# aikiriao/LINNE

Measured on AMD Instinct MI355X. Metric: frames/sec encode (-m 7) + decode, 44.1 kHz stereo, bit-exact; 1/2/4/8 GPU, higher is better.
Workload: dtype f64; 1 GPU; encode -m 7: 1 x 60 min 44.1 kHz int16 2-channel per GPU = 15504 frames of 10240 samples (tail 9280), MS on, PCM resident in HBM; decode = inverse hot path on the encode output; frames_per_gpu=15504, channels=2, preset=7, tracks_per_gpu=1

## Files before the change

linne_amd/csrc/lnn_dev_common.h:

```cpp
#ifndef LNN_DEV_COMMON_H_INCLUDED
#define LNN_DEV_COMMON_H_INCLUDED


#include "lnn_forms.h"
typedef double lnn_d2 __attribute__((ext_vector_type(2)));
typedef int lnn_v4i __attribute__((ext_vector_type(4)));

#ifdef LNN_TIMING_EXPERIMENTS
#define LNN_DBG_IS(p, v) ((p).dbg_maxtr == (v))
#define LNN_DBG_MAXTR(p) ((p).dbg_maxtr)
#else
#define LNN_DBG_IS(p, v) false
#define LNN_DBG_MAXTR(p) 0u
#endif
struct Plan {
    uint32_t C, S, bits, L, R, ms, F, J;
    uint32_t hist;
    uint32_t rows16;
    uint32_t search_long;
    uint32_t job_off;
    uint32_t prep_general;
    uint32_t prep_defer;
    uint32_t *prep_slow_n, *prep_slow_rows;
    uint32_t fused_last;
    RowRuns runs[2];
    uint32_t P[LNN_MAXL], coef_off[LNN_MAXL];
    double regs[LNN_MAXR];
    double scale;
    const int32_t *pcm; int32_t *resid; int32_t *prm; double *stats;
    uint32_t pcm16;
    const uint32_t *cls_of_frame; const uint32_t *frame_map; const DevClass *cls; const double *sintab; const double *wtab;
    int32_t *xint, *xtmp;
    double *sig;
    double *acorr;
    double *tcoef;
    double *ptail; uint8_t *ptail_set;
    double *tloss;
    double *tsum;
    uint32_t npart;
    double *txmax;
    double *thsum;
    uint8_t *uncertain;
    uint32_t *ucount;
    unsigned long long *min_margin;
    uint32_t dbg_maxtr;
    uint32_t force_exact;
    double *lparams;
    uint32_t *lunits;
    double *jloss, *jtail;
    const double *job_reg;
    const uint32_t *af_best; const double *af_loss;
    double *af_a;
    double *af_inv;
    double *af_R;
    uint32_t af_Rstride;
    double *af_rv, *af_invd;
    double *af_obj, *af_prev;
    uint32_t *af_state;
    uint32_t *af_prob, *af_nprob;
    double *af_pivot;
    double *capture;
};
#define LNN_CAP_WORDS   8

typedef const double __attribute__((address_space(4))) *lnn_cdp;

__device__ __forceinline__ int32_t pcm24_at(const void *base, size_t i)
{
    const uint8_t *b = (const uint8_t *)base + 3u * i;
    return (int32_t)((uint32_t)b[0] | ((uint32_t)b[1] << 8)) | ((int32_t)(int8_t)b[2] << 16);
}
__device__ __forceinline__ int32_t pcm_at(const Plan &p, size_t i) { return p.pcm16 == 1u ? (int32_t)((const int16_t *)p.pcm)[i] : (p.pcm16 == 2u ? pcm24_at(p.pcm, i) : p.pcm[i]); }

__device__ __forceinline__ double round_away(double d) { return (d >= 0.0) ? floor(d + 0.5) : -floor(-d + 0.5); }
__device__ __forceinline__ int32_t mulshr5(int32_t x, int32_t c) { return (int32_t)((uint32_t)x * (uint32_t)c) >> 5; }

__device__ void levinson(const double *r, double r0, uint32_t order, double *a, double *parcor_out)
{
    for (uint32_t i = 0; i < order + 2; i++) a[i] = 0.0;
    a[0] = 1.0;
    double ek = r0;
    a[1] = -r[1] / r0;
    if (parcor_out) parcor_out[0] = r[1] / ek;
    ek += r[1] * a[1];
    for (uint32_t k = 1; k < order; k++) {
        double gamma = 0.0;
        for (uint32_t i = 0; i < k + 1; i++) gamma += a[i] * r[k + 1 - i];
        gamma /= -ek;
        ek *= (1.0 - gamma * gamma);
        const double a0 = 1.0 + gamma * 0.0;
        const double ak1 = 0.0 + gamma * 1.0;
        uint32_t i = 1, j = k;
        while (i < j) {
            const double ai = a[i], aj = a[j];
            a[i] = ai + gamma * aj;
            a[j] = aj + gamma * ai;
            i++; j--;
        }
        if (i == j) { const double ai = a[i]; a[i] = ai + gamma * ai; }
        a[0] = a0; a[k + 1] = ak1;
        if (parcor_out) parcor_out[k] = -gamma;
    }
}


#endif
```

linne_amd/csrc/lnn_device.hip:

```cpp
#include <hip/hip_runtime.h>
#include <float.h>
#include <math.h>
#include <stdint.h>
#include <stdio.h>
#include <stdlib.h>
#include <string.h>
#include <atomic>
#include <new>
#include <vector>

#include "linne_amd.h"
#include "lnn_common.h"
#include "lnn_host.h"
#include "linne_decoder.h"
#include "linne_encoder.h"

#include "lnn_dev_common.h"
#include "lnn_k_prep.h"
#include "lnn_k_autocorr.h"
#include "lnn_k_levinson.h"
#include "lnn_k_fir.h"
#include "lnn_k_search.h"
#include "lnn_k_fwdloss.h"
#include "lnn_k_lastlayer.h"
#include "lnn_k_af.h"
#include "lnn_k_train.h"
#include "lnn_k_decode.h"
#include "lnn_k_decode_rows.h"
#include "lnn_k_decode_fused.h"
#include "lnn_k_finalize.h"
#include "lnn_k_rice.h"
#include "lnn_k_stream.h"
#include "lnn_k_index_batch.h"
#include "lnn_k_windows.h"
#include "lnn_k_stream_enc.h"
#include "lnn_stream_batch.h"
#include "lnn_k_splice.h"
static_assert(LINNE_AMD_T_IB_HEADERS == 69 && LINNE_AMD_T_IB_BEHIND == 70, "the index batch's timing kinds are 69 and 70");
static_assert(LINNE_AMD_SPLICE_T_COPY == 71 && LINNE_AMD_SPLICE_T_HEADER == 72, "the splice call's timing kinds are 71 and 72");
static_assert(LNN_FIR_TILE == FIR_TILE && LNN_FIR_WAVES == FIR_THREADS / 64 && LNN_SELW_MAXPART == SELW_MAXPART && LNN_SEARCH_JOB_MIN == SEARCH_JOB_MIN && LNN_LEV_MAXRIDE == LEV_MAXRIDE, "lnn_forms.h and the kernels disagree");

#define LNN_RICE_STREAMS 4
struct LINNEAmdContext {
    int device;
    hipStream_t stream; int own_stream;
    void *arena; uint64_t arena_bytes;
    char err[256];
    int timing;
    uint32_t na_max;
    hipEvent_t ev[2]; int ev_valid;
    hipEvent_t *span_ev; int *span_kind; int nspans, span_cap;
    uint32_t *d_ucount;
    hipStream_t sub[LNN_MAXSUB]; hipEvent_t sub_done[LNN_MAXSUB]; hipEvent_t ev_start; int nsub, nsub_forced ;
    int enc_streams_done;
    hipStream_t side; hipEvent_t side_done; int has_side;
    hipStream_t sib[2]; int sib1_tried;
    hipEvent_t fork_ev[LNN_MAXSUB], join_ev[LNN_MAXSUB], lev_fork_ev[LNN_MAXSUB], lev_join_ev[LNN_MAXSUB];
    DevClass *d_cls; double *d_sin; uint64_t sin_cap; double *d_wt; uint64_t wt_cap; uint32_t *d_clsidx; uint64_t clsidx_cap; uint32_t *d_map;    uint32_t *d_nsmp; uint64_t nsmp_cap;
    LnnClassTable tab;
    int last_search_form;
    const uint32_t *cur_idx;
    uint32_t *meta_h[LNN_META]; uint64_t meta_cap[LNN_META]; hipEvent_t meta_ev[LNN_META]; int meta_used[LNN_META]; int meta_next;
    hipStream_t copy_in, copy_out; int has_copy;
    hipStream_t rice_pool[LNN_RICE_STREAMS]; int n_rice_pool, rice_next;
    uint32_t *d_plan_nsmp; uint64_t plan_nsmp_cap; double rice_steps[32]; uint32_t rice_nsteps;
    int prod_ok;
    uint32_t learning;
    uint32_t af_iters;
    double *af_h; uint32_t af_h_cap;
    int pcm16_next;
    int capture_on;
    double *d_capture; uint64_t capture_cap, capture_n;
    void *sdec; uint64_t sdec_cap;
    void *senc; uint64_t senc_cap;
    void *wdec; uint64_t wdec_cap;
    void *wstage; uint64_t wstage_cap;
    int64_t senc_count[4];
    int64_t sbatch_count[3];
    void *xcand; uint64_t xcand_cap;
    int64_t ibatch_count[5];
    int span_keep;
    double rice_guard;
    void *hstage; uint64_t hstage_cap;
    void *spl; uint64_t spl_cap;
    void *spl_stage; uint64_t spl_stage_cap;
    int64_t splice_count[6];
    int outer_keep;
    LnnKnobs knob;
};

#define HIPCHK(ctx, call) do { hipError_t e_ = (call); if (e_ != hipSuccess) { snprintf((ctx)->err, sizeof((ctx)->err), "%s:%d %s -> %s", __FILE__, __LINE__, #call, hipGetErrorString(e_)); return LNN_NG; } } while (0)

static const uint32_t k_layers_a[] = { 2, 32 }, k_layers_b[] = { 4, 64, 8 }, k_layers_c[] = { 4, 128, 16 };
static const double k_regs_1[] = { 0.0 }, k_regs_2[] = { 0.0, 1.0 / 512.0 }, k_regs_4[] = { 0.0, 1.0 / 2048.0, 1.0 / 512.0, 1.0 / 128.0 };

extern "C" int lnn_preset_info(uint32_t preset, uint32_t *num_layers, uint32_t *layers, uint32_t *num_regs, double *regs)
{
    const uint32_t *L; const double *R; uint32_t nl, nr;
    if (preset >= 8) return -1;
    if (preset < 2) { L = k_layers_a; nl = 2; } else if (preset < 5) { L = k_layers_b; nl = 3; } else { L = k_layers_c; nl = 3; }
    switch (preset) { case 0: case 2: case 5: R = k_regs_1; nr = 1; break; case 1: case 3: case 6: R = k_regs_2; nr = 2; break; default: R = k_regs_4; nr = 4; }
    if (num_layers) *num_layers = nl;
    if (layers) for (uint32_t i = 0; i < nl; i++) layers[i] = L[i];
    if (num_regs) *num_regs = nr;
    if (regs) for (uint32_t i = 0; i < nr; i++) regs[i] = R[i];
    return 0;
}

__attribute__((constructor)) static void lnn_more_hw_queues(void) { setenv("GPU_MAX_HW_QUEUES", "8", 0); }

extern "C" int LINNEAmd_GetDeviceCount(void)
{
    int n = 0;
    if (hipGetDeviceCount(&n) != hipSuccess) return 0;
    return n;
}

static int ctx_encode_streams(LINNEAmdContext *ctx)
{
    if (ctx->enc_streams_done) return LNN_OK;
    ctx->enc_streams_done = 1;
    {
        int forced = 0;
        const int ns = lnn_context_streams(&forced);
        ctx->nsub_forced = forced;
        ctx->nsub = 0;
        for (int i = 0; i < ns; i++) {
            if (hipStreamCreateWithFlags(&ctx->sub[i], hipStreamNonBlocking) != hipSuccess || hipEventCreateWithFlags(&ctx->sub_done[i], hipEventDisableTiming) != hipSuccess) break;
            ctx->nsub++;
        }
        const bool have_start = hipEventCreateWithFlags(&ctx->ev_start, hipEventDisableTiming) == hipSuccess;
        if (!have_start) ctx->nsub = 0;
        ctx->has_side = have_start && hipStreamCreateWithFlags(&ctx->side, hipStreamNonBlocking) == hipSuccess
                && hipEventCreateWithFlags(&ctx->side_done, hipEventDisableTiming) == hipSuccess;
        for (int i = 0; i < LNN_MAXSUB && ctx->has_side; i++)
            ctx->has_side = hipEventCreateWithFlags(&ctx->fork_ev[i], hipEventDisableTiming) == hipSuccess
                    && hipEventCreateWithFlags(&ctx->join_ev[i], hipEventDisableTiming) == hipSuccess
                    && hipEventCreateWithFlags(&ctx->lev_fork_ev[i], hipEventDisableTiming) == hipSuccess
                    && hipEventCreateWithFlags(&ctx->lev_join_ev[i], hipEventDisableTiming) == hipSuccess;
        if (ctx->has_side) { ctx->sib[0] = ctx->side; ctx->sib[1] = ctx->side; }
    }
    return LNN_OK;
}

extern "C" struct LINNEAmdContext *LINNEAmd_ContextCreate(int device, uint64_t scratch_bytes)
{
    int n = 0;
    hipError_t e;
#define CC_FAIL(what) do { fprintf(stderr, "liblinne_amd: ContextCreate(device=%d): %s: %s\n", device, what, hipGetErrorString(e)); } while (0)
    if ((e = hipGetDeviceCount(&n)) != hipSuccess) { CC_FAIL("hipGetDeviceCount"); return NULL; }
    if (n <= 0 || device < 0 || device >= n) { fprintf(stderr, "liblinne_amd: ContextCreate(device=%d): %d HIP device(s) visible\n", device, n); return NULL; }
    if ((e = hipSetDevice(device)) != hipSuccess) { CC_FAIL("hipSetDevice"); return NULL; }
    LINNEAmdContext *ctx = (LINNEAmdContext *)calloc(1, sizeof(*ctx));
    if (!ctx) return NULL;
    ctx->device = device;
    if ((e = hipStreamCreateWithFlags(&ctx->stream, hipStreamNonBlocking)) != hipSuccess) { CC_FAIL("hipStreamCreate"); free(ctx); return NULL; }
    ctx->own_stream = 1;
    if (scratch_bytes == 0) scratch_bytes = 6ull << 30;
    if ((e = hipMalloc(&ctx->arena, scratch_bytes)) != hipSuccess) { CC_FAIL("hipMalloc(arena)"); hipStreamDestroy(ctx->stream); free(ctx); return NULL; }
    ctx->arena_bytes = scratch_bytes;
    if ((e = hipMalloc((void **)&ctx->d_cls, sizeof(DevClass) * LNN_MAXCLS)) != hipSuccess) { CC_FAIL("hipMalloc(classes)"); hipFree(ctx->arena); hipStreamDestroy(ctx->stream); free(ctx); return NULL; }
    if ((e = hipMalloc((void **)&ctx->d_ucount, 4 * sizeof(uint32_t))) != hipSuccess) { CC_FAIL("hipMalloc(counter)"); }
    lnn_knobs_read_context(&ctx->knob); ctx->last_search_form = -1;
    (void)hipFuncSetAttribute((const void *)k_levinson_lds, hipFuncAttributeMaxDynamicSharedMemorySize, (int)LEV_LDS_BUDGET);
    (void)hipFuncSetAttribute((const void *)k_synth_pipe, hipFuncAttributeMaxDynamicSharedMemorySize, (int)LEV_LDS_BUDGET);
    if ((e = hipEventCreate(&ctx->ev[0])) != hipSuccess || (e = hipEventCreate(&ctx->ev[1])) != hipSuccess) { CC_FAIL("hipEventCreate"); }
#undef CC_FAIL
    return ctx;
}

extern "C" void LINNEAmd_ContextDestroy(struct LINNEAmdContext *ctx)
{
    if (!ctx) return;
    hipSetDevice(ctx->device);
    hipStreamSynchronize(ctx->stream);
    if (ctx->arena) hipFree(ctx->arena);
    if (ctx->d_cls) hipFree(ctx->d_cls);
    if (ctx->d_ucount) hipFree(ctx->d_ucount);
    if (ctx->d_capture) hipFree(ctx->d_capture);
    for (int i = 0; i < ctx->nsub; i++) { hipStreamSynchronize(ctx->sub[i]); hipStreamDestroy(ctx->sub[i]); hipEventDestroy(ctx->sub_done[i]); }
    if (ctx->ev_start) hipEventDestroy(ctx->ev_start);
    if (ctx->has_side && ctx->sib[1] != ctx->side) { hipStreamSynchronize(ctx->sib[1]); hipStreamDestroy(ctx->sib[1]); }
    if (ctx->has_side) { hipStreamSynchronize(ctx->side); hipStreamDestroy(ctx->side); hipEventDestroy(ctx->side_done); }
    for (int i = 0; i < LNN_MAXSUB; i++) {
        if (ctx->fork_ev[i]) hipEventDestroy(ctx->fork_ev[i]);
        if (ctx->join_ev[i]) hipEventDestroy(ctx->join_ev[i]);
        if (ctx->lev_fork_ev[i]) hipEventDestroy(ctx->lev_fork_ev[i]);
        if (ctx->lev_join_ev[i]) hipEventDestroy(ctx->lev_join_ev[i]);
    }
    if (ctx->d_sin) hipFree(ctx->d_sin);
    if (ctx->d_wt) hipFree(ctx->d_wt);
    if (ctx->d_clsidx) hipFree(ctx->d_clsidx);
    if (ctx->d_nsmp) hipFree(ctx->d_nsmp);
    if (ctx->d_plan_nsmp) hipFree(ctx->d_plan_nsmp);
    if (ctx->hstage) hipFree(ctx->hstage);
    if (ctx->sdec) hipFree(ctx->sdec);
    if (ctx->senc) hipFree(ctx->senc);
    if (ctx->wdec) hipFree(ctx->wdec);
    if (ctx->xcand) hipFree(ctx->xcand);
    if (ctx->spl) hipFree(ctx->spl);
    if (ctx->spl_stage) hipHostFree(ctx->spl_stage);
    if (ctx->wstage) hipHostFree(ctx->wstage);
    if (ctx->af_h) hipHostFree(ctx->af_h);
    for (int i = 0; i < LNN_META; i++) { if (ctx->meta_h[i]) hipHostFree(ctx->meta_h[i]); if (ctx->meta_ev[i]) hipEventDestroy(ctx->meta_ev[i]); }
    for (int i = 0; i < ctx->n_rice_pool; i++) { hipStreamSynchronize(ctx->rice_pool[i]); hipStreamDestroy(ctx->rice_pool[i]); }
    if (ctx->has_copy) { hipStreamSynchronize(ctx->copy_in); hipStreamSynchronize(ctx->copy_out); hipStreamDestroy(ctx->copy_in); hipStreamDestroy(ctx->copy_out); }
    hipEventDestroy(ctx->ev[0]); hipEventDestroy(ctx->ev[1]);
    for (int i = 0; i < 2 * ctx->span_cap; i++) hipEventDestroy(ctx->span_ev[i]);
    free(ctx->span_ev); free(ctx->span_kind);
    if (ctx->own_stream) hipStreamDestroy(ctx->stream);
    free(ctx);
}

extern "C" const char *LINNEAmd_GetLastError(const struct LINNEAmdContext *ctx) { return ctx ? ctx->err : "no context"; }

extern "C" int LINNEAmd_SetStream(struct LINNEAmdContext *ctx, void *hip_stream)
{
    if (!ctx) return LNN_INVALID_ARGUMENT;
    HIPCHK(ctx, hipSetDevice(ctx->device));
    HIPCHK(ctx, hipStreamSynchronize(ctx->stream));
    if (ctx->own_stream) { HIPCHK(ctx, hipStreamDestroy(ctx->stream)); ctx->own_stream = 0; }
    ctx->stream = (hipStream_t)hip_stream;
    return LNN_OK;
}

extern "C" int LINNEAmd_ReserveScratch(struct LINNEAmdContext *ctx, uint64_t bytes)
{
    if (!ctx) return LNN_INVALID_ARGUMENT;
    if (ctx->arena_bytes >= bytes) return LNN_OK;
    HIPCHK(ctx, hipSetDevice(ctx->device));
    HIPCHK(ctx, hipStreamSynchronize(ctx->stream));
    void *fresh = NULL;
    if (hipMalloc(&fresh, bytes) != hipSuccess) { (void)hipGetLastError(); snprintf(ctx->err, sizeof(ctx->err), "cannot reserve %llu bytes of scratch", (unsigned long long)bytes); return LNN_NG; }
    if (ctx->arena) HIPCHK(ctx, hipFree(ctx->arena));
    ctx->arena = fresh; ctx->arena_bytes = bytes;
    return LNN_OK;
}

extern "C" int64_t LINNEAmd_GetLastFallbackCount(struct LINNEAmdContext *ctx)
{
    if (!ctx) return -1;
    uint32_t v = 0;
    if (hipSetDevice(ctx->device) != hipSuccess || hipStreamSynchronize(ctx->stream) != hipSuccess
            || hipMemcpy(&v, ctx->d_ucount, sizeof(v), hipMemcpyDeviceToHost) != hipSuccess) return -1;
    return (int64_t)v;
}

extern "C" double LINNEAmd_GetLastMinMargin(struct LINNEAmdContext *ctx)
{
    if (!ctx) return -1.0;
    double v = -1.0;
    if (hipSetDevice(ctx->device) != hipSuccess || hipStreamSynchronize(ctx->stream) != hipSuccess
            || hipMemcpy(&v, ctx->d_ucount + 2, sizeof(v), hipMemcpyDeviceToHost) != hipSuccess) return -1.0;
    return v;
}

extern "C" int LINNEAmd_SetSearchCapture(struct LINNEAmdContext *ctx, int enable)
{
    if (!ctx) return LNN_INVALID_ARGUMENT;
    ctx->capture_on = enable ? 1 : 0;
    return LNN_OK;
}

extern "C" int64_t LINNEAmd_GetLastSearchCapture(struct LINNEAmdContext *ctx, double *host, uint64_t capacity_records)
{
    if (!ctx) return -1;
    const uint64_t n = ctx->capture_n < capacity_records ? ctx->capture_n : capacity_records;
    if (hipSetDevice(ctx->device) != hipSuccess || hipStreamSynchronize(ctx->stream) != hipSuccess) return -1;
    if (n && (!host || hipMemcpy(host, ctx->d_capture, n * LNN_CAP_WORDS * sizeof(double), hipMemcpyDeviceToHost) != hipSuccess)) return -1;
    return (int64_t)ctx->capture_n;
}

extern "C" int LINNEAmd_Synchronize(struct LINNEAmdContext *ctx)
{
    if (!ctx) return LNN_INVALID_ARGUMENT;
    HIPCHK(ctx, hipSetDevice(ctx->device));
    HIPCHK(ctx, hipStreamSynchronize(ctx->stream));
    return LNN_OK;
}

extern "C" int LINNEAmd_SetLearning(struct LINNEAmdContext *ctx, uint32_t enable)
{
    if (!ctx) return LNN_INVALID_ARGUMENT;
    ctx->learning = enable ? 1u : 0u;
    return LNN_OK;
}
extern "C" int LINNEAmd_SetAfIterations(struct LINNEAmdContext *ctx, uint32_t iterations)
{
    if (!ctx) return LNN_INVALID_ARGUMENT;
    ctx->af_iters = iterations;
    return LNN_OK;
}
extern "C" int LINNEAmd_EnableTiming(struct LINNEAmdContext *ctx, int enable) { if (!ctx) return LNN_INVALID_ARGUMENT; ctx->timing = enable; return LNN_OK; }
static int span_begin(LINNEAmdContext *ctx, int kind, hipStream_t st)
{
    if (!ctx->timing) return -1;
    if (ctx->nspans == ctx->span_cap) {
        const int ncap = ctx->span_cap ? ctx->span_cap * 2 : 256;
        hipEvent_t *ne = (hipEvent_t *)realloc(ctx->span_ev, sizeof(hipEvent_t) * 2 * ncap);
        if (!ne) return -1;
        ctx->span_ev = ne;
        int *nk = (int *)realloc(ctx->span_kind, sizeof(int) * ncap);
        if (!nk) return -1;
        ctx->span_kind = nk;
        for (int i = 2 * ctx->span_cap; i < 2 * ncap; i++) if (hipEventCreate(&ctx->span_ev[i]) != hipSuccess) return -1;
        ctx->span_cap = ncap;
    }
    const int id = ctx->nspans++;
    ctx->span_kind[id] = kind;
    (void)hipEventRecord(ctx->span_ev[2 * id], st);
    return id;
}
static void span_end(LINNEAmdContext *ctx, int id, hipStream_t st) { if (id >= 0) (void)hipEventRecord(ctx->span_ev[2 * id + 1], st); }

extern "C" double LINNEAmd_GetLastTimingMs(struct LINNEAmdContext *ctx, int which)
{
    if (!ctx || which < 0) return -1.0;
    if (which == 0) {
        float ms = -1.0f;
        if (!ctx->ev_valid) return -1.0;
        if (hipEventSynchronize(ctx->ev[1]) != hipSuccess || hipEventElapsedTime(&ms, ctx->ev[0], ctx->ev[1]) != hipSuccess) return -1.0;
        return ms;
    }
    double sum = 0.0; int cnt = 0;
    for (int i = 0; i < ctx->nspans; i++) if (ctx->span_kind[i] == which) {
        float ms = 0.0f;
        if (hipEventSynchronize(ctx->span_ev[2 * i + 1]) != hipSuccess || hipEventElapsedTime(&ms, ctx->span_ev[2 * i], ctx->span_ev[2 * i + 1]) != hipSuccess) return -1.0;
        sum += ms; cnt++;
    }
    return cnt ? sum : -1.0;
}
extern "C" int LINNEAmd_GetLastSearchLongForm(struct LINNEAmdContext *ctx) { return ctx ? ctx->last_search_form : -1; }
extern "C" int LINNEAmd_GetLastTimingLaunches(struct LINNEAmdContext *ctx, int which)
{
    if (!ctx) return 0;
    int cnt = 0;
    for (int i = 0; i < ctx->nspans; i++) if (ctx->span_kind[i] == which) cnt++;
    return cnt;
}

static int ensure_buf(LINNEAmdContext *ctx, void **ptr, uint64_t *cap, uint64_t need)
{
    if (*cap >= need) return LNN_OK;
    HIPCHK(ctx, hipStreamSynchronize(ctx->stream));
    if (*ptr) HIPCHK(ctx, hipFree(*ptr));
    *ptr = NULL; *cap = 0;
    HIPCHK(ctx, hipMalloc(ptr, need));
    *cap = need;
    return LNN_OK;
}

static int shape_info(const struct LINNEAmdShape *s, HostShape *h)
{
    if (!s || s->preset >= 8 || s->num_channels == 0 || s->num_channels > LNN_MAXCH || s->bits_per_sample == 0 || s->bits_per_sample > 32
            || s->num_samples_per_block == 0 || s->ch_process_method > 1 || (s->ch_process_method == 1 && s->num_channels < 2)) return LNN_INVALID_FORMAT;
    lnn_preset_info(s->preset, &h->L, h->P, &h->R, h->regs);
    uint32_t off = 0; h->maxP = 0;
    for (uint32_t l = 0; l < h->L; l++) { h->coef_off[l] = off; off += h->P[l]; if (h->P[l] > h->maxP) h->maxP = h->P[l]; }
    for (uint32_t l = 0; l < h->L; l++) if (s->num_samples_per_block <= h->P[l]) return LNN_INVALID_FORMAT;
    return LNN_OK;
}

static int meta_acquire(LINNEAmdContext *ctx, uint32_t F, int *m_out)
{
    const int m = ctx->meta_next;
    ctx->meta_next = (m + 1) % LNN_META;
    if (ctx->meta_used[m]) { HIPCHK(ctx, hipEventSynchronize(ctx->meta_ev[m])); ctx->meta_used[m] = 0; }
    if (!ctx->meta_ev[m]) HIPCHK(ctx, hipEventCreateWithFlags(&ctx->meta_ev[m], hipEventDisableTiming));
    if (ctx->meta_cap[m] < 4ull * F) {
        const uint64_t cap = 4ull * (F < 4096u ? 4096u : F);
        if (ctx->meta_h[m]) { HIPCHK(ctx, hipHostFree(ctx->meta_h[m])); ctx->meta_h[m] = NULL; ctx->meta_cap[m] = 0; }
        HIPCHK(ctx, hipHostMalloc((void **)&ctx->meta_h[m], sizeof(uint32_t) * cap, hipHostMallocDefault));
        ctx->meta_cap[m] = cap;
    }
    *m_out = m;
    return LNN_OK;
}

static int copy_lengths(LINNEAmdContext *ctx, const struct LINNEAmdShape *shape, const uint32_t *h_num_samples, uint32_t F, uint32_t *dst)
{
    const uint32_t S = shape->num_samples_per_block;
    for (uint32_t f = 0; f < F; f++) {
        const uint32_t n = h_num_samples ? h_num_samples[f] : S;
        if (n == 0 || n > S) { snprintf(ctx->err, sizeof(ctx->err), "frame %u: num_samples %u out of range", f, n); return LNN_INVALID_ARGUMENT; }
        dst[f] = n;
    }
    return LNN_OK;
}

static int upload_lengths(LINNEAmdContext *ctx, const struct LINNEAmdShape *shape, const uint32_t *h_num_samples, uint32_t F)
{
    int m, ret;
    if ((ret = meta_acquire(ctx, F, &m)) != LNN_OK) return ret;
    uint32_t *nsm = ctx->meta_h[m];
    if ((ret = copy_lengths(ctx, shape, h_num_samples, F, nsm)) != LNN_OK) return ret;
    if ((ret = ensure_buf(ctx, (void **)&ctx->d_nsmp, &ctx->nsmp_cap, sizeof(uint32_t) * (uint64_t)(F ? F : 1))) != LNN_OK) return ret;
    HIPCHK(ctx, hipMemcpyAsync(ctx->d_nsmp, nsm, sizeof(uint32_t) * F, hipMemcpyHostToDevice, ctx->stream));
    HIPCHK(ctx, hipEventRecord(ctx->meta_ev[m], ctx->stream));
    ctx->meta_used[m] = 1;
    return LNN_OK;
}

extern "C" double lnn_welch_divisor(uint32_t unit_samples) { return lnn_welch_div(unit_samples); }
extern "C" double lnn_sin_window(uint32_t s, uint32_t n) { return sin((3.1415926535897932384626433832795029 * s) / (n - 1)); }
extern "C" double lnn_cholesky_pivot(double sum) { return pow(sum, -0.5); }

static int build_classes(LINNEAmdContext *ctx, const struct LINNEAmdShape *shape, const HostShape *hs,
        const uint32_t *h_num_samples, uint32_t F)
{
    int m, ret;
    { const int r_ = meta_acquire(ctx, F, &m); if (r_ != LNN_OK) return r_; }
    uint32_t *idx = ctx->meta_h[m], *map = ctx->meta_h[m] + F, *raw = ctx->meta_h[m] + 2 * (size_t)F;
    ctx->cur_idx = idx;
    LnnClassTable &tab = ctx->tab;
    LnnCallClasses cc;
    switch (lnn_call_classes(&tab, shape, hs, &ctx->knob, h_num_samples, F, idx, map, raw, &cc)) {
    case LNN_CLS_BAD_LENGTH: snprintf(ctx->err, sizeof(ctx->err), "frame %u: num_samples %u out of range", cc.error_frame, h_num_samples[cc.error_frame]); return LNN_INVALID_ARGUMENT;
    case LNN_CLS_TOO_MANY: snprintf(ctx->err, sizeof(ctx->err), "more than %d distinct frame lengths in one batch", LNN_MAXCLS); return LNN_INVALID_ARGUMENT;
    default: break;
    }
    ctx->na_max = cc.na_max; ctx->prod_ok = cc.prod_ok;
    if (cc.branch != LNN_CLS_REUSE) {
        const uint64_t sin_total = tab.sin_total, wt_total = tab.wt_total;
        double *sintab = (double *)malloc(sizeof(double) * (sin_total ? sin_total : 1));
        double *wt = (double *)calloc(wt_total ? wt_total : 1, sizeof(double));
        if (!sintab || !wt) { free(sintab); free(wt); tab.valid = 0; tab.ncls = 0; snprintf(ctx->err, sizeof(ctx->err), "out of host memory"); return LNN_NG; }
        for (uint32_t k = 0; k < tab.ncls; k++) {
            const DevClass &c = tab.cls[k];
            const uint32_t n = c.n;
            for (uint32_t s = 0; s < n; s++) sintab[c.sin_off + s] = lnn_sin_window(s, n);
            for (uint32_t l = 0; l < hs->L; l++)
                for (uint32_t t = 0; t < c.ntrials[l]; t++) {
                    const uint32_t u = c.trial_u[l][t], nu = c.na / u;
                    const double div = c.trial_div[l][t];
                    double *w = wt + c.wt_off[l][t];
                    for (uint32_t loc = 0; loc < nu; loc++) {
                        const uint32_t h = (loc < (nu >> 1)) ? loc : (nu - 1 - loc);
                        w[loc] = div * (double)h * (double)(nu - 1 - h);
                    }
                }
        }
        hipError_t e = hipDeviceSynchronize();
        ret = (e == hipSuccess) ? ensure_buf(ctx, (void **)&ctx->d_sin, &ctx->sin_cap, sizeof(double) * (sin_total ? sin_total : 1)) : LNN_NG;
        if (ret == LNN_OK) ret = ensure_buf(ctx, (void **)&ctx->d_wt, &ctx->wt_cap, sizeof(double) * (wt_total ? wt_total : 1));
        if (ret != LNN_OK) { free(sintab); free(wt); tab.valid = 0; tab.ncls = 0; return ret; }
        e = hipMemcpyAsync(ctx->d_sin, sintab, sizeof(double) * sin_total, hipMemcpyHostToDevice, ctx->stream);
        if (e == hipSuccess) e = hipMemcpyAsync(ctx->d_wt, wt, sizeof(double) * wt_total, hipMemcpyHostToDevice, ctx->stream);
        if (e == hipSuccess) e = hipMemcpyAsync(ctx->d_cls, tab.cls, sizeof(DevClass) * LNN_MAXCLS, hipMemcpyHostToDevice, ctx->stream);
        if (e == hipSuccess) e = hipStreamSynchronize(ctx->stream);
        free(sintab); free(wt);
        if (e != hipSuccess) { tab.valid = 0; tab.ncls = 0; snprintf(ctx->err, sizeof(ctx->err), "class table upload: %s", hipGetErrorString(e)); return LNN_NG; }
    }
    if ((ret = ensure_buf(ctx, (void **)&ctx->d_clsidx, &ctx->clsidx_cap, sizeof(uint32_t) * 2 * (uint64_t)(F ? F : 1))) != LNN_OK) return ret;
    ctx->d_map = ctx->d_clsidx + F;
    HIPCHK(ctx, hipMemcpyAsync(ctx->d_clsidx, idx, sizeof(uint32_t) * 2 * (size_t)F, hipMemcpyHostToDevice, ctx->stream));
    HIPCHK(ctx, hipEventRecord(ctx->meta_ev[m], ctx->stream));
    ctx->meta_used[m] = 1;
    return LNN_OK;
}

static uint64_t align_up(uint64_t v) { return (v + 255u) & ~(uint64_t)255u; }

static uint64_t frame_scratch_bytes(const struct LINNEAmdShape *shape, const HostShape *hs, uint32_t af_iters = 0, uint32_t learning = 0)
{
    const uint64_t C = shape->num_channels, S = shape->num_samples_per_block, J = C * hs->R;
    uint64_t b = 0;
    b += 2 * C * S * sizeof(int32_t);
    b += J * 2 * S * sizeof(double);
    b += J * LNN_MAXT * LNN_ACW * sizeof(double);
    b += J * LNN_MAXT * LNN_MAXP * sizeof(double);
    b += J * LNN_MAXT * LNN_MAXU * (sizeof(double) + 1);
    b += J * LNN_MAXT * sizeof(double) * (1 + (uint64_t)((S + FIR_TILE - 1) / FIR_TILE) * (FIR_THREADS / 64)) + J;
    b += J * sizeof(double) * (uint64_t)((S + FIR_TILE - 1) / FIR_TILE) * (FIR_THREADS / 64) + 256;
    b += J * LNN_MAXT * sizeof(double) + 256;
    b += J * LNN_MAXL * LNN_MAXP * sizeof(double);
    b += J * LNN_MAXL * sizeof(uint32_t);
    b += J * 2 * sizeof(double);
    b += C * sizeof(uint32_t) + 512;
    if (af_iters)
        b += C * (sizeof(double) * ((uint64_t)hs->maxP * hs->maxP + S + 3 * LNN_MAXP + 3 * LNN_MAXU + 2) + sizeof(uint32_t) * (2 * LNN_MAXU + 1)) + 8192;
    if (af_iters || learning) b += C * (sizeof(uint32_t) + 2 * sizeof(double)) + 1024;
    if (learning)
        b += C * (sizeof(double) * ((2 + LNN_MAXL) * S + 2 * LNN_MAXL * LNN_MAXP + 2) + sizeof(uint32_t)) + 4096;
    return b + 4096;
}

extern "C" uint64_t LINNEAmd_ScratchBytesPerFrame(const struct LINNEAmdShape *shape)
{
    HostShape hs;
    if (shape_info(shape, &hs) != LNN_OK) return 0;
    return frame_scratch_bytes(shape, &hs);
}

#define LNN_BY_ORDER(P_, LAUNCH_) do { switch (P_) { case 2: LAUNCH_(2); break; case 4: LAUNCH_(4); break; case 8: LAUNCH_(8); break; default: LAUNCH_(16); break; } } while (0)
#define LNN_BY_L0_SPEC(l0_, spec_, LAUNCH_) do { if (l0_) { if (spec_) LAUNCH_(true, true); else LAUNCH_(true, false); } else { if (spec_) LAUNCH_(false, true); else LAUNCH_(false, false); } } while (0)

template <int MODE> static void launch_fir(hipStream_t st, const Plan &p, uint32_t l, uint32_t cur, uint32_t J, uint32_t grid_y, bool spec)
{
    const dim3 grid(J, grid_y), blk(FIR_THREADS);
#define LNN_F2(L0_, SPEC_) hipLaunchKernelGGL((k_fir2<MODE, L0_, SPEC_>), grid, blk, 0, st, p, l, cur)
    LNN_BY_L0_SPEC(l == 0, spec, LNN_F2);
#undef LNN_F2
}

template <int PP> static void launch_fir_small_p(hipStream_t st, const Plan &p, uint32_t l, uint32_t cur, const dim3 grid, bool spec)
{
#define LNN_FS(L0_, SPEC_) hipLaunchKernelGGL((k_fir_small<PP, L0_, SPEC_>), grid, dim3(FIR_THREADS), 0, st, p, l, cur)
    LNN_BY_L0_SPEC(l == 0, spec, LNN_FS);
#undef LNN_FS
}
static void launch_fir_small_search(hipStream_t st, const Plan &p, uint32_t l, uint32_t cur, uint32_t J, uint32_t tiles, bool spec, uint32_t P)
{
    const dim3 grid(l == 0 ? J / p.R : J, tiles);
#define LNN_FSP(PP_) launch_fir_small_p<PP_>(st, p, l, cur, grid, spec)
    LNN_BY_ORDER(P, LNN_FSP);
#undef LNN_FSP
}

static void launch_last_layer(hipStream_t st, const Plan &q, uint32_t l, uint32_t cur, uint32_t J)
{
#define LNN_LL(PP_) hipLaunchKernelGGL(k_last_layer<PP_>, dim3((J + 63) / 64), dim3(64), 0, st, q, l, cur)
    LNN_BY_ORDER(q.P[l], LNN_LL);
#undef LNN_LL
}

static void launch_fwd_loss(hipStream_t st, const Plan &q, uint32_t l, uint32_t cur, uint32_t J, bool mw)
{
    const dim3 g((J + 63) / 64);
#define LNN_FLM(PP_) hipLaunchKernelGGL(k_fwd_loss_mw<PP_>, g, dim3(320), 0, st, q, l, cur)
#define LNN_FL(PP_) hipLaunchKernelGGL(k_fwd_loss<PP_>, g, dim3(64), 0, st, q, l, cur)
    if (mw) LNN_BY_ORDER(q.P[l], LNN_FLM); else LNN_BY_ORDER(q.P[l], LNN_FL);
#undef LNN_FLM
#undef LNN_FL
}

static void launch_search_long(hipStream_t st, const Plan &q, uint32_t l, uint32_t cur, uint32_t J, uint32_t tiles, int form)
{
    const dim3 grid(J, form == 2 ? 1u : tiles), blk(FIR_THREADS);
#define LNN_SL(TWO_, JOB_) do { if (q.P[l] == 128u) hipLaunchKernelGGL((k_search_long<128, TWO_, JOB_>), grid, blk, 0, st, q, l, cur); else hipLaunchKernelGGL((k_search_long<64, TWO_, JOB_>), grid, blk, 0, st, q, l, cur); } while (0)
    if (form == 2) LNN_SL(true, true); else if (form == 1) LNN_SL(true, false); else LNN_SL(false, false);
#undef LNN_SL
}

struct EncodeCall {
    const struct LINNEAmdShape *shape; HostShape hs; uint32_t C, S, num_frames, pcm16;
    const int32_t *d_pcm; int32_t *d_residual, *d_params; double *d_stats;
    LnnSplit split;
};
struct Chunk {
    LINNEAmdContext *ctx; hipStream_t st; const HostShape *hs;
    hipStream_t sib; uint32_t slot;
    uint32_t C, S, f0, Fc; uint64_t CF, J;
    const uint32_t *idx;
    Plan p; LnnChunkForms forms;
    uint8_t *abase; uint64_t part_bytes;
    uint32_t *af_best; double *af_loss, *af_reg; TrainArgs tr;
};
struct Pass {
    const Plan *q; const LnnChunkForms *forms; uint32_t J, af_iters;
    uint32_t cur;
};

static void fill_plan(Plan &p, const EncodeCall &e, uint32_t F)
{
    memset(&p, 0, sizeof(p));
    p.C = e.C; p.S = e.S; p.bits = e.shape->bits_per_sample; p.L = e.hs.L; p.R = e.hs.R; p.F = F;
    for (uint32_t l = 0; l < e.hs.L; l++) p.P[l] = e.hs.P[l];
    p.scale = ldexp(1.0, -(int)(e.shape->bits_per_sample - 1));
    p.pcm = e.d_pcm; p.pcm16 = e.pcm16; p.stats = e.d_stats;
}

static int launch_stats(LINNEAmdContext *ctx, const EncodeCall &e)
{
    Plan ps; fill_plan(ps, e, e.num_frames);
    ps.cls_of_frame = ctx->d_clsidx; ps.frame_map = ctx->d_map; ps.cls = ctx->d_cls; ps.sintab = ctx->d_sin;
    hipStream_t ss = ctx->stream;
    if (ctx->has_side) { ss = ctx->side; HIPCHK(ctx, hipStreamWaitEvent(ss, ctx->ev_start, 0)); }
    if (!ctx->knob.nostats) {
        const int sp_ = span_begin(ctx, LINNE_AMD_T_STATS, ss);
        if (lnn_stats_rows_form(&ctx->knob, e.num_frames, e.C, e.S, e.hs.P[0])) {
            const dim3 g((e.num_frames * e.C + 63u) / 64u);
#define LNN_SR(W_, T_) do { if (e.pcm16 == 1u) hipLaunchKernelGGL((k_stats_rows<W_, 1>), g, dim3(T_), 0, ss, ps); else if (e.pcm16 == 2u) hipLaunchKernelGGL((k_stats_rows<W_, 2>), g, dim3(T_), 0, ss, ps); else hipLaunchKernelGGL((k_stats_rows<W_, 0>), g, dim3(T_), 0, ss, ps); } while (0)
            if (e.hs.P[0] == 4u) LNN_SR(5, 320); else LNN_SR(3, 192);
#undef LNN_SR
        }
        else hipLaunchKernelGGL(k_stats, dim3(e.num_frames, e.C), dim3(STAT_THREADS), 0, ss, ps);
        span_end(ctx, sp_, ss);
    }
    if (ss != ctx->stream) HIPCHK(ctx, hipEventRecord(ctx->side_done, ss));
    return LNN_OK;
}

static int chunk_setup(Chunk &k, LINNEAmdContext *ctx, const EncodeCall &e, uint32_t f0, uint32_t slot)
{
    const uint32_t S = e.S;
    k.ctx = ctx; k.hs = &e.hs; k.C = e.C; k.S = S; k.f0 = f0;
    k.st = e.split.use_sub ? ctx->sub[slot] : ctx->stream;
    k.slot = slot; k.sib = ctx->sib[slot & 1u];
    k.Fc = (e.num_frames - f0 < e.split.chunk) ? (e.num_frames - f0) : (uint32_t)e.split.chunk;
    k.CF = (uint64_t)k.Fc * e.C; k.J = k.CF * e.hs.R;
    k.idx = ctx->cur_idx + f0;
    const uint64_t CF = k.CF, J = k.J;
    const LnnChunkIn in = { &e.hs, e.C, S, k.Fc, ctx->tab.cls, k.idx, &ctx->knob, e.split.use_sub, ctx->has_side != 0, ctx->af_iters, ctx->learning, false };
    lnn_chunk_forms(&in, &k.forms);
    Plan &p = k.p;
    fill_plan(p, e, k.Fc);
    p.ms = e.shape->ch_process_method; p.J = (uint32_t)J;
    for (uint32_t l = 0; l < e.hs.L; l++) p.coef_off[l] = e.hs.coef_off[l];
    for (uint32_t r = 0; r < e.hs.R; r++) p.regs[r] = e.hs.regs[r];
    p.resid = e.d_residual; p.prm = e.d_params;
    p.fused_last = k.forms.fuse_cfg ? 1u : 0u;
    p.search_long = ctx->knob.search_long ? 1u : 0u;
    p.rows16 = ctx->knob.rows16 ? 1u : 0u;
    p.prep_general = ctx->knob.prep_general ? 1u : 0u;
    p.prep_defer = k.forms.prep_defer ? 1u : 0u;
    lnn_build_runs(&p.runs[0], k.idx, k.Fc, e.C); lnn_build_runs(&p.runs[1], k.idx, k.Fc, e.C * e.hs.R);
    p.hist = k.forms.hist ? 1u : 0u;
    p.cls_of_frame = ctx->d_clsidx + f0; p.frame_map = ctx->d_map + f0; p.cls = ctx->d_cls; p.sintab = ctx->d_sin; p.wtab = ctx->d_wt; p.ucount = ctx->d_ucount; p.min_margin = (unsigned long long *)(ctx->d_ucount + 2); p.force_exact = ctx->knob.force_exact ? 1u : 0u; p.dbg_maxtr = ctx->knob.dbg_maxtr;
    p.capture = ctx->capture_n ? ctx->d_capture : NULL;
    k.part_bytes = e.split.part_bytes;
    k.abase = (uint8_t *)ctx->arena + (size_t)slot * k.part_bytes;
    uint8_t *a = k.abase;
#define TAKE(ptr, type, count) do { ptr = (type *)a; a += align_up(sizeof(type) * (uint64_t)(count)); } while (0)
    TAKE(p.xint, int32_t, CF * S); TAKE(p.xtmp, int32_t, CF * S);
    TAKE(p.sig, double, J * 2 * S);
    TAKE(p.acorr, double, J * LNN_MAXT * LNN_ACW); TAKE(p.tcoef, double, J * LNN_MAXT * LNN_MAXP);
    TAKE(p.ptail, double, J * LNN_MAXT * LNN_MAXU); TAKE(p.ptail_set, uint8_t, J * LNN_MAXT * LNN_MAXU);
    TAKE(p.tloss, double, J * LNN_MAXT); p.npart = ((S + FIR_TILE - 1) / FIR_TILE) * (FIR_THREADS / 64); TAKE(p.tsum, double, J * LNN_MAXT * p.npart); TAKE(p.txmax, double, J * p.npart); TAKE(p.thsum, double, J * LNN_MAXT); TAKE(p.uncertain, uint8_t, J); TAKE(p.lparams, double, J * LNN_MAXL * LNN_MAXP);
    TAKE(p.lunits, uint32_t, J * LNN_MAXL); TAKE(p.jloss, double, J); TAKE(p.jtail, double, J);
    TAKE(p.prep_slow_n, uint32_t, 64); TAKE(p.prep_slow_rows, uint32_t, CF);
    k.af_best = NULL; k.af_loss = NULL; k.af_reg = NULL;
    memset(&k.tr, 0, sizeof(k.tr));
    TrainArgs &tr = k.tr;
    if (ctx->af_iters || ctx->learning) { TAKE(k.af_best, uint32_t, CF); TAKE(k.af_loss, double, CF); TAKE(k.af_reg, double, CF); }
    if (ctx->learning) {
        TAKE(tr.buf, double, CF * TR_NBUF * S); TAKE(tr.dparams, double, CF * LNN_MAXL * LNN_MAXP); TAKE(tr.momentum, double, CF * LNN_MAXL * LNN_MAXP);
        TAKE(tr.loss, double, CF); TAKE(tr.prev, double, CF); TAKE(tr.active, uint32_t, CF); TAKE(tr.nactive, uint32_t, 64);
    }
    if (ctx->af_iters) {
        TAKE(p.af_a, double, CF * LNN_MAXP); TAKE(p.af_inv, double, CF * S); p.af_Rstride = e.hs.maxP * e.hs.maxP; TAKE(p.af_R, double, CF * p.af_Rstride);
        TAKE(p.af_rv, double, CF * LNN_MAXP); TAKE(p.af_invd, double, CF * LNN_MAXP);
        TAKE(p.af_obj, double, CF * LNN_MAXU); TAKE(p.af_prev, double, CF * LNN_MAXU); TAKE(p.af_state, uint32_t, CF * LNN_MAXU);
        TAKE(p.af_prob, uint32_t, CF * LNN_MAXU); TAKE(p.af_nprob, uint32_t, 64); TAKE(p.af_pivot, double, CF * LNN_MAXU);
    }
#undef TAKE
    if ((uint64_t)(a - k.abase) > k.part_bytes) { snprintf(ctx->err, sizeof(ctx->err), "internal: arena overflow"); return LNN_NG; }
    return LNN_OK;
}

static int launch_prep(Chunk &k)
{
    LINNEAmdContext *ctx = k.ctx; hipStream_t st = k.st; const Plan &p = k.p;
    if (p.prep_defer) HIPCHK(ctx, hipMemsetAsync(p.prep_slow_n, 0, sizeof(uint32_t), st));
    const int sp_ = span_begin(ctx, LINNE_AMD_T_PREP, st);
    hipLaunchKernelGGL(k_prep, dim3(k.Fc, k.C), dim3(PREP_THREADS), 0, st, p);
    if (p.prep_defer) hipLaunchKernelGGL(k_prep_slow, dim3((uint32_t)((k.CF + 63) / 64)), dim3(256), 0, st, p);
    span_end(ctx, sp_, st);
    return LNN_OK;
}

static void sibling_for_levinson(Chunk &k)
{
    LINNEAmdContext *ctx = k.ctx;
    if ((k.slot & 1u) && ctx->sib[1] == ctx->side && !ctx->sib1_tried) {
        ctx->sib1_tried = 1;
        if (hipStreamCreateWithFlags(&ctx->sib[1], hipStreamNonBlocking) != hipSuccess) { (void)hipGetLastError(); ctx->sib[1] = ctx->side; }
    }
    k.sib = ctx->sib[k.slot & 1u];
}

static int launch_lags(Chunk &k, const Pass &ps, uint32_t l)
{
    LINNEAmdContext *ctx = k.ctx; hipStream_t st = k.st; const Plan &q = *ps.q; const LnnLayerForms &lf = ps.forms->layer[l];
    const uint32_t P = k.hs->P[l];
    if (lf.lev_beside && !lf.lev_inline) sibling_for_levinson(k);
    if (lf.beside) {
        HIPCHK(ctx, hipEventRecord(ctx->fork_ev[k.slot], st)); HIPCHK(ctx, hipStreamWaitEvent(k.sib, ctx->fork_ev[k.slot], 0));
        const int sp_ = span_begin(ctx, LINNE_AMD_T_AUTOCORR, k.sib); dispatch_autocorr2(k.sib, q, l, ps.cur, ctx->na_max, (ctx->prod_ok >> l) & 1); span_end(ctx, sp_, k.sib);
        HIPCHK(ctx, hipEventRecord(ctx->join_ev[k.slot], k.sib));
    }
    if (lf.hist_layer) {
        for (int w = 0; w < 3; w++) {
            if (P == 64u && w == 1) continue;
            const int sp_ = span_begin(ctx, LINNE_AMD_T_HIST_P + w, st); (void)launch_autocorr_hist(st, q, l, ps.cur, w, w == 2 && lf.lev_beside); span_end(ctx, sp_, st);
            if (w == 0 && lf.lev_beside) {
                const LnnLevLaunch &v = lf.lev[0];
                const hipStream_t ls = lf.lev_inline ? st : k.sib;
                if (lf.lev_inline && lf.beside) HIPCHK(ctx, hipStreamWaitEvent(st, ctx->join_ev[k.slot], 0));
                if (!lf.lev_inline) { HIPCHK(ctx, hipEventRecord(ctx->lev_fork_ev[k.slot], st)); HIPCHK(ctx, hipStreamWaitEvent(k.sib, ctx->lev_fork_ev[k.slot], 0)); }
                hipLaunchKernelGGL(k_levinson_lds, dim3((ps.J + 63) / 64, v.u), dim3(v.threads), v.lds, ls, q, l, v.t, v.ride);
                if (!lf.lev_inline) HIPCHK(ctx, hipEventRecord(ctx->lev_join_ev[k.slot], k.sib));
            }
        }
    }
    if (lf.beside) HIPCHK(ctx, hipStreamWaitEvent(st, ctx->join_ev[k.slot], 0));
    else if (!lf.hist_all) {
        const int sp_ = span_begin(ctx, (P >= 32u) ? LINNE_AMD_T_AUTOCORR : LINNE_AMD_T_AUTOCORR_SHORT, st); dispatch_autocorr2(st, q, l, ps.cur, ctx->na_max, (ctx->prod_ok >> l) & 1); span_end(ctx, sp_, st);
    }
    return LNN_OK;
}

static void launch_levinson(Chunk &k, const Pass &ps, uint32_t l)
{
    LINNEAmdContext *ctx = k.ctx; hipStream_t st = k.st; const Plan &q = *ps.q; const LnnLayerForms &lf = ps.forms->layer[l];
    const uint32_t P = k.hs->P[l], maxu = P < 128u ? P : 128u;
    if (lf.lev_beside && !lf.lev_inline) (void)hipStreamWaitEvent(st, ctx->lev_join_ev[k.slot], 0);
    const int sp_ = span_begin(ctx, LINNE_AMD_T_LEVINSON, st);
    if (lf.lev_wave) hipLaunchKernelGGL(k_levinson_wave, dim3(ps.J, 2u * maxu - 1u), dim3(64), 0, st, q, l);
    else for (uint32_t i = lf.lev_beside ? 1u : 0u; i < lf.nlev; i++) {
        const LnnLevLaunch &v = lf.lev[i];
        hipLaunchKernelGGL(k_levinson_lds, dim3((ps.J + 63) / 64, v.u), dim3(v.threads), v.lds, st, q, l, v.t, v.ride);
    }
    span_end(ctx, sp_, st);
}

static void launch_search(Chunk &k, const Pass &ps, uint32_t l)
{
    LINNEAmdContext *ctx = k.ctx; hipStream_t st = k.st; const Plan &q = *ps.q; const LnnLayerForms &lf = ps.forms->layer[l];
    const uint32_t tiles = (k.S + FIR_TILE - 1) / FIR_TILE;
    if (lf.long_any) {
        const int sp_ = span_begin(ctx, LINNE_AMD_T_SEARCH_LONG, st);
        ctx->last_search_form = lf.search_form == 2 ? 1 : 0;
        launch_search_long(st, q, l, ps.cur, ps.J, tiles, lf.search_form);
        span_end(ctx, sp_, st);
    }
    if (lf.long_any && lf.long_all) return;
    const int sp_ = span_begin(ctx, (l == 0) ? LINNE_AMD_T_SEARCH_L0 : (lf.fir_spec ? LINNE_AMD_T_SEARCH : LINNE_AMD_T_SEARCH_PLAIN), st);
    if (lf.fir_small) launch_fir_small_search(st, q, l, ps.cur, ps.J, tiles, lf.fir_spec, k.hs->P[l]);
    else if (lf.long_any) {
        const uint32_t rpf = ps.J / k.Fc;
        for (uint32_t f = 0, g = 0; lnn_next_left_run(&lf, k.idx, k.Fc, g, &f, &g); ) {
            Plan qq = q; qq.job_off = f * rpf;
            launch_fir<2>(st, qq, l, ps.cur, (g - f) * rpf, tiles, lf.fir_spec);
        }
    }
    else launch_fir<2>(st, q, l, ps.cur, ps.J, tiles, lf.fir_spec);
    span_end(ctx, sp_, st);
}

static void launch_select(Chunk &k, const Pass &ps, uint32_t l)
{
    LINNEAmdContext *ctx = k.ctx; hipStream_t st = k.st; const Plan &q = *ps.q; const LnnLayerForms &lf = ps.forms->layer[l];
    for (uint32_t exact = 0; exact < 2; exact++) {
        const int sp_ = span_begin(ctx, exact ? LINNE_AMD_T_EXACT : LINNE_AMD_T_SELECT, st);
        if (exact) { if (l == 0) hipLaunchKernelGGL((k_fir2<0, true, false>), dim3(ps.J, 1), dim3(FIR_THREADS), 0, st, q, l, ps.cur); else hipLaunchKernelGGL((k_fir2<0, false, false>), dim3(ps.J, 1), dim3(FIR_THREADS), 0, st, q, l, ps.cur); }
        if (lf.sel_wave) hipLaunchKernelGGL(k_select_wave, dim3(ps.J), dim3(64), 0, st, q, l, exact);
        else hipLaunchKernelGGL(k_select, dim3((ps.J + 63) / 64), dim3(64), 0, st, q, l, exact);
        span_end(ctx, sp_, st);
    }
}

static int run_af(Chunk &k, const Pass &ps, uint32_t l)
{
    LINNEAmdContext *ctx = k.ctx; hipStream_t st = k.st; const Plan &q = *ps.q;
    const uint32_t P = k.hs->P[l], S = k.S, Jq = ps.J, cur = ps.cur;
    HIPCHK(ctx, hipMemsetAsync(q.af_nprob, 0, sizeof(uint32_t), st));
    hipLaunchKernelGGL(k_af_init, dim3((Jq + 255) / 256), dim3(256), 0, st, q, l);
    uint32_t nprob = 0;
    HIPCHK(ctx, hipMemcpyAsync(&nprob, q.af_nprob, sizeof(uint32_t), hipMemcpyDeviceToHost, st));
    HIPCHK(ctx, hipStreamSynchronize(st));
    if (nprob == 0) return LNN_OK;
    if (ctx->af_h_cap < nprob) {
        if (ctx->af_h) HIPCHK(ctx, hipHostFree(ctx->af_h));
        ctx->af_h = NULL; ctx->af_h_cap = 0;
        HIPCHK(ctx, hipHostMalloc((void **)&ctx->af_h, sizeof(double) * (size_t)nprob, hipHostMallocDefault));
        ctx->af_h_cap = nprob;
    }
    uint32_t mblocks = 0;
    for (uint32_t uu = 1; uu <= P; uu <<= 1) { const uint32_t b_ = uu * afm_blocks_per_unit(P / uu); if (b_ > mblocks) mblocks = b_; }
    for (uint32_t it = 0; it < ps.af_iters; it++) {
        hipLaunchKernelGGL(k_af_resid, dim3(Jq, (S + AFR_THREADS * 4 - 1) / (AFR_THREADS * 4)), dim3(AFR_THREADS), 0, st, q, l, cur);
        hipLaunchKernelGGL(k_af_obj, dim3(nprob), dim3(64), 0, st, q, l, cur);
        hipLaunchKernelGGL(k_af_matrix, dim3(Jq, mblocks), dim3(AFM_THREADS), 0, st, q, l, cur);
        for (uint32_t i = 0; i < P; i++) {
            hipLaunchKernelGGL(k_af_pivot, dim3((nprob + 63) / 64), dim3(64), 0, st, q, l, i);
            HIPCHK(ctx, hipMemcpyAsync(ctx->af_h, q.af_pivot, sizeof(double) * (size_t)nprob, hipMemcpyDeviceToHost, st));
            HIPCHK(ctx, hipStreamSynchronize(st));
            for (uint32_t j = 0; j < nprob; j++) { const double v = ctx->af_h[j]; ctx->af_h[j] = (v <= 0.0) ? -1.0 : lnn_cholesky_pivot(v); }
            HIPCHK(ctx, hipMemcpyAsync(q.af_pivot, ctx->af_h, sizeof(double) * (size_t)nprob, hipMemcpyHostToDevice, st));
            hipLaunchKernelGGL(k_af_column, dim3(nprob), dim3(128), 0, st, q, l, i);
        }
        hipLaunchKernelGGL(k_af_solve, dim3((nprob + 63) / 64), dim3(64), 0, st, q, l);
    }
    hipLaunchKernelGGL(k_af_finish, dim3((Jq + 255) / 256), dim3(256), 0, st, q, l);
    HIPCHK(ctx, hipGetLastError());
    return LNN_OK;
}

static int run_layers(Chunk &k, Pass &ps)
{
    LINNEAmdContext *ctx = k.ctx; hipStream_t st = k.st; const Plan &q = *ps.q;
    const uint32_t L = k.hs->L, tiles = (k.S + FIR_TILE - 1) / FIR_TILE;
    int ret;
    ps.cur = 0;
    for (uint32_t l = 0; l < L; l++) {
        const LnnLayerForms &lf = ps.forms->layer[l];
        if ((ret = launch_lags(k, ps, l)) != LNN_OK) return ret;
        launch_levinson(k, ps, l);
        if (lf.last_layer) {
            { const int sp_ = span_begin(ctx, LINNE_AMD_T_FWD_LOSS, st); launch_last_layer(st, q, l, ps.cur, ps.J); span_end(ctx, sp_, st); }
            { const int sp_ = span_begin(ctx, LINNE_AMD_T_SELECT, st); hipLaunchKernelGGL(k_select, dim3((ps.J + 63) / 64), dim3(64), 0, st, q, l, 2u); span_end(ctx, sp_, st); }
        } else {
            launch_search(k, ps, l);
            launch_select(k, ps, l);
            if (lf.fwd_loss) { const int sp_ = span_begin(ctx, LINNE_AMD_T_FWD_LOSS, st); launch_fwd_loss(st, q, l, ps.cur, ps.J, lf.fwd_loss_mw); span_end(ctx, sp_, st); }
        }
        if (ps.af_iters && (ret = run_af(k, ps, l)) != LNN_OK) return ret;
        if (lf.forward) {
            const int sp_ = span_begin(ctx, (l == 0) ? LINNE_AMD_T_FORWARD_L0 : (lf.fir_spec ? LINNE_AMD_T_FORWARD : LINNE_AMD_T_FORWARD_PLAIN), st);
            launch_fir<1>(st, q, l, ps.cur, ps.J, lf.forward_walk ? 1u : tiles, lf.fir_spec);
            span_end(ctx, sp_, st);
        }
        ps.cur ^= 1u;
    }
    return LNN_OK;
}

static int run_train(Chunk &k, const Plan &q, const uint32_t *best)
{
    LINNEAmdContext *ctx = k.ctx; hipStream_t st = k.st; TrainArgs &tr = k.tr;
    const uint32_t CF = (uint32_t)k.CF, L = k.hs->L;
    tr.p = q; tr.best = best; tr.CF = CF;
    const uint32_t tiles = (k.S + TR_TILE - 1) / TR_TILE;
    const int sp_ = span_begin(ctx, LINNE_AMD_T_TRAIN, st);
    hipLaunchKernelGGL(k_tr_init, dim3((CF + 255) / 256), dim3(256), 0, st, tr);
    for (uint32_t it = 0; it < 2000u; it++) {
        HIPCHK(ctx, hipMemsetAsync(tr.nactive, 0, sizeof(uint32_t), st));
        for (uint32_t l = 0; l < L; l++) hipLaunchKernelGGL(k_tr_forward, dim3(CF, tiles), dim3(TR_THREADS), 0, st, tr, l);
        hipLaunchKernelGGL(k_tr_loss, dim3(CF), dim3(64), 0, st, tr);
        for (uint32_t l = L - 1; l >= 1; l--) hipLaunchKernelGGL(k_tr_back, dim3(CF, tiles), dim3(TR_THREADS), 0, st, tr, l);
        hipLaunchKernelGGL(k_tr_gradp, dim3(CF, L), dim3(128), 0, st, tr);
        hipLaunchKernelGGL(k_tr_update, dim3(CF), dim3(128), 0, st, tr, (double)0.8f, (double)0.1f, 1.0e-7);
        uint32_t left = 0;
        HIPCHK(ctx, hipMemcpyAsync(&left, tr.nactive, sizeof(uint32_t), hipMemcpyDeviceToHost, st));
        HIPCHK(ctx, hipStreamSynchronize(st));
        if (left == 0) break;
    }
    span_end(ctx, sp_, st);
    HIPCHK(ctx, hipGetLastError());
    return LNN_OK;
}

static void launch_finish(Chunk &k, const Plan &q)
{
    const uint32_t CF = (uint32_t)k.CF;
    const int sp_ = span_begin(k.ctx, LINNE_AMD_T_FINALIZE, k.st);
    hipLaunchKernelGGL(k_quantize, dim3(CF), dim3(64), 0, k.st, q);
    hipLaunchKernelGGL(k_fir_cascade, dim3(CF, k.forms.cascade_walk ? 1u : (k.S + FIN_TILE - 1) / FIN_TILE), dim3(FIN_THREADS), 0, k.st, q);
    span_end(k.ctx, sp_, k.st);
}

static int run_final_pass(Chunk &k)
{
    LINNEAmdContext *ctx = k.ctx; hipStream_t st = k.st; const Plan &p = k.p;
    const uint32_t CF = (uint32_t)k.CF;
    int ret;
    Plan q = p;
    q.R = 1; q.J = CF; q.regs[0] = 0.0;
    q.hist = 0; q.fused_last = 0; q.search_long = 0;
    q.capture = NULL;
    lnn_build_runs(&q.runs[1], k.idx, k.Fc, k.C);
    q.job_reg = k.af_reg; q.af_best = k.af_best; q.af_loss = k.af_loss;
    hipLaunchKernelGGL(k_af_best, dim3((CF + 255) / 256), dim3(256), 0, st, p, k.af_best, k.af_loss, k.af_reg);
    const LnnChunkIn in = { k.hs, k.C, k.S, k.Fc, ctx->tab.cls, k.idx, &ctx->knob, false, ctx->has_side != 0, ctx->af_iters, ctx->learning, true };
    LnnChunkForms ff;
    lnn_chunk_forms(&in, &ff);
    Pass fp = { &q, &ff, CF, ctx->af_iters, 0 };
    const int sp_ = span_begin(ctx, LINNE_AMD_T_AF_PASS, st);
    if ((ret = run_layers(k, fp)) != LNN_OK) return ret;
    span_end(ctx, sp_, st);
    if (ctx->learning && (ret = run_train(k, q, NULL)) != LNN_OK) return ret;
    launch_finish(k, q);
    return LNN_OK;
}

static int enqueue_chunk(Chunk &k)
{
    LINNEAmdContext *ctx = k.ctx; hipStream_t st = k.st; const Plan &p = k.p;
    int ret;
    if ((ret = launch_prep(k)) != LNN_OK) return ret;
    Pass sp = { &p, &k.forms, (uint32_t)k.J, 0u, 0 };
    if ((ret = run_layers(k, sp)) != LNN_OK) return ret;
    if (k.forms.chain_sum) {
        const int sp_ = span_begin(ctx, LINNE_AMD_T_FINAL_LOSS, st);
        if (k.forms.chain_sum_wave) hipLaunchKernelGGL(k_chain_sum_wave<1>, dim3((uint32_t)k.J), dim3(64), 0, st, p, 0u, sp.cur);
        else hipLaunchKernelGGL(k_chain_sum<1>, dim3(((uint32_t)k.J + 63) / 64), dim3(SUM_THREADS), 0, st, p, 0u, sp.cur);
        span_end(ctx, sp_, st);
    }
    if (ctx->af_iters) { if ((ret = run_final_pass(k)) != LNN_OK) return ret; }
    else {
        if (ctx->learning) {
            hipLaunchKernelGGL(k_af_best, dim3(((uint32_t)k.CF + 255) / 256), dim3(256), 0, st, p, k.af_best, k.af_loss, k.af_reg);
            if ((ret = run_train(k, p, k.af_best)) != LNN_OK) return ret;
        }
        launch_finish(k, p);
    }
    HIPCHK(ctx, hipGetLastError());
    return LNN_OK;
}

static int enqueue_chunks(LINNEAmdContext *ctx, const EncodeCall &e)
{
    uint32_t chunk_index = 0;
    for (uint32_t f0 = 0; f0 < e.num_frames; f0 += (uint32_t)e.split.chunk, chunk_index++) {
        Chunk k;
        int ret = chunk_setup(k, ctx, e, f0, chunk_index % e.split.nsub);
        if (ret == LNN_OK) ret = enqueue_chunk(k);
        if (ret != LNN_OK) return ret;
    }
    return LNN_OK;
}

extern "C" int LINNEAmd_EncodeFramesDevice(struct LINNEAmdContext *ctx, const struct LINNEAmdShape *shape,
        const int32_t *d_pcm, const uint32_t *h_num_samples, uint32_t num_frames,
        int32_t *d_residual, int32_t *d_params, double *d_stats)
{
    if (!ctx) return LNN_INVALID_ARGUMENT;
    ctx->err[0] = 0;
    EncodeCall e;
    e.pcm16 = (uint32_t)ctx->pcm16_next;
    ctx->pcm16_next = 0;
    if (!shape || !d_pcm || !d_residual || !d_params || !d_stats) { snprintf(ctx->err, sizeof(ctx->err), "null argument"); return LNN_INVALID_ARGUMENT; }
    if (num_frames == 0) return LNN_OK;
    int ret = shape_info(shape, &e.hs);
    if (ret != LNN_OK) { snprintf(ctx->err, sizeof(ctx->err), "invalid shape"); return ret; }
    e.shape = shape; e.C = shape->num_channels; e.S = shape->num_samples_per_block; e.num_frames = num_frames;
    e.d_pcm = d_pcm; e.d_residual = d_residual; e.d_params = d_params; e.d_stats = d_stats;
    HIPCHK(ctx, hipSetDevice(ctx->device));
    if ((ret = ctx_encode_streams(ctx)) != LNN_OK) return ret;
    lnn_knobs_read_call(&ctx->knob);
    if ((ret = build_classes(ctx, shape, &e.hs, h_num_samples, num_frames)) != LNN_OK) return ret;
    const uint64_t per_frame = frame_scratch_bytes(shape, &e.hs, ctx->af_iters, ctx->learning);
    if (ctx->arena_bytes < per_frame * 4 + 65536) {
        HIPCHK(ctx, hipStreamSynchronize(ctx->stream));
        HIPCHK(ctx, hipFree(ctx->arena)); ctx->arena = NULL; ctx->arena_bytes = 0;
        HIPCHK(ctx, hipMalloc(&ctx->arena, per_frame * 4 + 65536));
        ctx->arena_bytes = per_frame * 4 + 65536;
    }
    e.split = lnn_call_split(ctx->arena_bytes, per_frame, num_frames, e.C, e.hs.R, ctx->nsub, ctx->nsub_forced != 0, &ctx->knob);
    const LnnSplit &sp = e.split;
    if (!ctx->span_keep) ctx->nspans = 0;
    ctx->last_search_form = -1;
    ctx->capture_n = 0;
    if (ctx->capture_on) {
        const uint64_t nrec = (uint64_t)num_frames * e.C * e.hs.R * e.hs.L * LNN_MAXT;
        if (ctx->capture_cap < nrec) {
            HIPCHK(ctx, hipStreamSynchronize(ctx->stream));
            if (ctx->d_capture) HIPCHK(ctx, hipFree(ctx->d_capture));
            ctx->d_capture = NULL; ctx->capture_cap = 0;
            HIPCHK(ctx, hipMalloc((void **)&ctx->d_capture, nrec * LNN_CAP_WORDS * sizeof(double)));
            ctx->capture_cap = nrec;
        }
        HIPCHK(ctx, hipMemsetAsync(ctx->d_capture, 0xFF, nrec * LNN_CAP_WORDS * sizeof(double), ctx->stream));
        ctx->capture_n = nrec;
    }
    HIPCHK(ctx, hipMemsetAsync(ctx->d_ucount, 0, sizeof(uint32_t), ctx->stream));
    HIPCHK(ctx, hipMemsetAsync(ctx->d_ucount + 2, 0x7F, 2 * sizeof(uint32_t), ctx->stream));
    if (ctx->timing && !ctx->span_keep) { HIPCHK(ctx, hipEventRecord(ctx->ev[0], ctx->stream)); }
    if (sp.use_sub || ctx->has_side) HIPCHK(ctx, hipEventRecord(ctx->ev_start, ctx->stream));
    if (sp.use_sub) for (uint32_t i = 0; i < sp.nsub; i++) HIPCHK(ctx, hipStreamWaitEvent(ctx->sub[i], ctx->ev_start, 0));
    if ((ret = launch_stats(ctx, e)) != LNN_OK) return ret;
    const int loop_ret = enqueue_chunks(ctx, e);
    if (loop_ret != LNN_OK) {
        if (sp.use_sub) for (uint32_t i = 0; i < sp.nsub; i++) (void)hipStreamSynchronize(ctx->sub[i]);
        if (ctx->has_side) { (void)hipStreamSynchronize(ctx->side); (void)hipStreamSynchronize(ctx->sib[1]); }
        return loop_ret;
    }
    if (ctx->has_side) HIPCHK(ctx, hipStreamWaitEvent(ctx->stream, ctx->side_done, 0));
    if (sp.use_sub) {
        for (uint32_t i = 0; i < sp.nsub; i++) { HIPCHK(ctx, hipEventRecord(ctx->sub_done[i], ctx->sub[i])); HIPCHK(ctx, hipStreamWaitEvent(ctx->stream, ctx->sub_done[i], 0)); }
    }
    if (ctx->timing) { HIPCHK(ctx, hipEventRecord(ctx->ev[1], ctx->stream)); ctx->ev_valid = 1; }
    return LNN_OK;
}

static int params_in_range(LINNEAmdContext *ctx, const HostShape *hs, uint32_t C, const int32_t *h_params, uint32_t num_frames)
{
    uint32_t ncoef = 0;
    for (uint32_t l = 0; l < hs->L; l++) ncoef += hs->P[l];
    const uint64_t rows = (uint64_t)num_frames * C;
    uint32_t bad = 0;
    for (uint64_t r = 0; r < rows; r++) {
        const int32_t *c = h_params + r * LINNE_AMD_PARAM_WORDS + LINNE_AMD_PRM_COEF;
        uint32_t acc = 0;
        for (uint32_t i = 0; i < ncoef; i++) acc |= (uint32_t)(c[i] + 128) & ~255u;
        bad |= acc;
    }
    if (bad) { snprintf(ctx->err, sizeof(ctx->err), "a coefficient outside [-128, 127] in the parameter records (not a LINNE stream's)"); return LNN_INVALID_FORMAT; }
    return LNN_OK;
}

static void launch_synth_rows(hipStream_t st, const DecPlan &p, uint32_t l, const LnnDecLayer &d, uint32_t CF)
{
    const dim3 grows((CF + 3) / 4), grows8((CF + 7) / 8), b(64);
    if (d.form == LNN_DL_ROWS8) switch (d.pb) {
    case 4: hipLaunchKernelGGL((k_synth_rows8<4>), grows8, b, 0, st, p, l); break;
    case 8: hipLaunchKernelGGL((k_synth_rows8<8>), grows8, b, 0, st, p, l); break;
    default: hipLaunchKernelGGL((k_synth_rows8<16>), grows8, b, 0, st, p, l); break;
    }
    else switch (d.nch) {
    case 0: if (d.pb == 4u) hipLaunchKernelGGL((k_synth_rows<0, 4>), grows, b, 0, st, p, l); else hipLaunchKernelGGL((k_synth_rows<0>), grows, b, 0, st, p, l); break;
    case 1: hipLaunchKernelGGL((k_synth_rows<1>), grows, b, 0, st, p, l); break;
    case 3: hipLaunchKernelGGL((k_synth_rows<3>), grows, b, 0, st, p, l); break;
    default: hipLaunchKernelGGL((k_synth_rows<7>), grows, b, 0, st, p, l); break;
    }
}
template <int PP> static void launch_synth_small_p(hipStream_t st, const DecPlan &p, uint32_t l, bool de, uint32_t CF)
{
    if (de) hipLaunchKernelGGL((k_synth_small<PP, true>), dim3((CF + 63) / 64), dim3(64), 0, st, p, l); else hipLaunchKernelGGL((k_synth_small<PP, false>), dim3((CF + 63) / 64), dim3(64), 0, st, p, l);
}
static void launch_synth_lanes(hipStream_t st, const DecPlan &p, uint32_t l, const LnnDecLayer &d, uint32_t CF)
{
#define LNN_SS(PP_) launch_synth_small_p<PP_>(st, p, l, d.de, CF)
    if (d.form == LNN_DL_SMALL) LNN_BY_ORDER(d.pb, LNN_SS);
#undef LNN_SS
    else if (d.form == LNN_DL_BIG) switch (d.pb) {
    case 32:  hipLaunchKernelGGL((k_synth_big<32>), dim3((CF + 15) / 16), dim3(64), 0, st, p, l); break;
    case 64:  hipLaunchKernelGGL((k_synth_big<64>), dim3((CF + 15) / 16), dim3(64), 0, st, p, l); break;
    default: hipLaunchKernelGGL((k_synth_big<128>), dim3((CF + 15) / 16), dim3(64), 0, st, p, l); break;
    }
    else hipLaunchKernelGGL(k_synthesize, dim3(CF), dim3(64), 0, st, p, l, 0u);
}

static int decode_frames_dev(LINNEAmdContext *ctx, const struct LINNEAmdShape *shape, const HostShape &hs,
        int32_t *d_data, const uint32_t *d_nsmp, uint32_t num_frames, const int32_t *d_params)
{
    DecPlan p; memset(&p, 0, sizeof(p));
    p.C = shape->num_channels; p.S = shape->num_samples_per_block; p.L = hs.L; p.ms = shape->ch_process_method; p.F = num_frames;
    for (uint32_t l = 0; l < hs.L; l++) { p.P[l] = hs.P[l]; p.coef_off[l] = hs.coef_off[l]; }
    p.data = d_data; p.prm = d_params; p.nsmp = d_nsmp;
    hipStream_t st = ctx->stream;
    const uint32_t CF = num_frames * p.C, gsmall = (CF + 63) / 64;
    if (hs.P[0] > 16) { snprintf(ctx->err, sizeof(ctx->err), "internal: layer 0 of order %u", hs.P[0]); return LNN_NG; }
    LnnDecodeForms df;
    lnn_decode_forms(&hs, p.C, p.S, p.ms, num_frames, ((uintptr_t)d_data & 15u) == 0u, SP_LDS_BYTES(p.S) <= LEV_LDS_BUDGET, &ctx->knob, &df);
    if (df.call == LNN_DEC_PIPE) { const int sp_ = span_begin(ctx, LINNE_AMD_T_SYNTH_PIPE, st); hipLaunchKernelGGL(k_synth_pipe, dim3(CF), dim3(64 * (hs.L + 1)), SP_LDS_BYTES(p.S), st, p); span_end(ctx, sp_, st); }
    else if (df.call == LNN_DEC_WAVE) { const int sp_ = span_begin(ctx, LINNE_AMD_T_SYNTH, st); hipLaunchKernelGGL(k_synthesize, dim3(CF), dim3(64), 0, st, p, 0xFFFFFFFFu, 1u); span_end(ctx, sp_, st); }
    else for (int32_t li = (int32_t)hs.L - 1; li >= 0; li--) {
        const uint32_t l = (uint32_t)li;
        const LnnDecLayer &d = df.layer[l];
        if (d.form == LNN_DL_FUSED_L0) {
            const int sp_ = span_begin(ctx, LINNE_AMD_T_SYNTH_L0_DE, st);
            if (d.ms_fold) hipLaunchKernelGGL((k_synth_l0_de<true>), dim3(gsmall), dim3(64 * SF_WAVES), 0, st, p); else hipLaunchKernelGGL((k_synth_l0_de<false>), dim3(gsmall), dim3(64 * SF_WAVES), 0, st, p);
            span_end(ctx, sp_, st);
        } else if (d.form == LNN_DL_ROWS || d.form == LNN_DL_ROWS8) {
            const int sp_ = span_begin(ctx, d.nch > 0 ? LINNE_AMD_T_SYNTH_ROWS : LINNE_AMD_T_SYNTH_ROWS_SHORT, st);
            launch_synth_rows(st, p, l, d, CF);
            span_end(ctx, sp_, st);
            if (d.de) {
                const int sd_ = span_begin(ctx, LINNE_AMD_T_DEEMPH_LR, st);
                if (d.ms_fold) hipLaunchKernelGGL((k_deemph_lr<true>), dim3(gsmall), dim3(64 * (2 + DL_STORERS)), 0, st, p); else hipLaunchKernelGGL((k_deemph_lr<false>), dim3(gsmall), dim3(64 * (2 + DL_STORERS)), 0, st, p);
                span_end(ctx, sd_, st);
            }
        } else {
            const int sp_ = span_begin(ctx, d.form == LNN_DL_SMALL ? LINNE_AMD_T_SYNTH_SMALL : (d.form == LNN_DL_BIG ? LINNE_AMD_T_SYNTH_BIG : LINNE_AMD_T_SYNTH), st);
            launch_synth_lanes(st, p, l, d, CF);
            span_end(ctx, sp_, st);
        }
    }
    if (df.ms_separate)
        { const int sp_ = span_begin(ctx, LINNE_AMD_T_MS_TO_LR, st); hipLaunchKernelGGL(k_ms_to_lr, dim3(num_frames, (p.S + 255) / 256), dim3(256), 0, st, p); span_end(ctx, sp_, st); }
    HIPCHK(ctx, hipGetLastError());
    if (ctx->timing) { HIPCHK(ctx, hipEventRecord(ctx->ev[1], ctx->stream)); ctx->ev_valid = 1; }
    return LNN_OK;
}

extern "C" int LINNEAmd_DecodeFramesDevice(struct LINNEAmdContext *ctx, const struct LINNEAmdShape *shape,
        int32_t *d_data, const uint32_t *h_num_samples, uint32_t num_frames, const int32_t *d_params)
{
    if (!ctx) return LNN_INVALID_ARGUMENT;
    ctx->err[0] = 0;
    if (!shape || !d_data || !d_params) { snprintf(ctx->err, sizeof(ctx->err), "null argument"); return LNN_INVALID_ARGUMENT; }
    if (num_frames == 0) return LNN_OK;
    HostShape hs;
    int ret = shape_info(shape, &hs);
    if (ret != LNN_OK) { snprintf(ctx->err, sizeof(ctx->err), "invalid shape"); return ret; }
    HIPCHK(ctx, hipSetDevice(ctx->device));
    lnn_knobs_read_call(&ctx->knob);
    if ((ret = upload_lengths(ctx, shape, h_num_samples, num_frames)) != LNN_OK) return ret;
    ctx->nspans = 0;
    if (ctx->timing) { HIPCHK(ctx, hipEventRecord(ctx->ev[0], ctx->stream)); }
    return decode_frames_dev(ctx, shape, hs, d_data, ctx->d_nsmp, num_frames, d_params);
}

#define HSTAGE_KEEP ((uint64_t)64 << 20)
static int hstage_get(LINNEAmdContext *ctx, uint64_t bytes, void **out, int *transient)
{
    *transient = 0;
    if (bytes > HSTAGE_KEEP) {
        if (hipMalloc(out, bytes) != hipSuccess) { (void)hipGetLastError(); snprintf(ctx->err, sizeof(ctx->err), "hipMalloc of staging buffers failed"); return LNN_NG; }
        *transient = 1;
        return LNN_OK;
    }
    if (ctx->hstage_cap < bytes) {
        HIPCHK(ctx, hipStreamSynchronize(ctx->stream));
        if (ctx->hstage) { HIPCHK(ctx, hipFree(ctx->hstage)); ctx->hstage = NULL; ctx->hstage_cap = 0; }
        uint64_t cap = bytes < ((uint64_t)1 << 20) ? ((uint64_t)1 << 20) : bytes;
        if (hipMalloc(&ctx->hstage, cap) != hipSuccess) { (void)hipGetLastError(); ctx->hstage = NULL; snprintf(ctx->err, sizeof(ctx->err), "hipMalloc of staging buffers failed"); return LNN_NG; }
        ctx->hstage_cap = cap;
    }
    *out = ctx->hstage;
    return LNN_OK;
}

extern "C" int LINNEAmd_EncodeFramesHost(struct LINNEAmdContext *ctx, const struct LINNEAmdShape *shape,
        const int32_t *pcm, const uint32_t *num_samples, uint32_t num_frames,
        int32_t *residual, int32_t *params, double *stats)
{
    if (!ctx) return LNN_INVALID_ARGUMENT;
    if (!shape || !pcm || !residual || !params || !stats) return LNN_INVALID_ARGUMENT;
    if (num_frames == 0) return LNN_OK;
    HIPCHK(ctx, hipSetDevice(ctx->device));
    const uint64_t CS = (uint64_t)shape->num_channels * shape->num_samples_per_block;
    const uint64_t nb = sizeof(int32_t) * CS * num_frames, pb = sizeof(int32_t) * LINNE_AMD_PARAM_WORDS * (uint64_t)shape->num_channels * num_frames,
                   sb = sizeof(double) * LINNE_AMD_STAT_WORDS * (uint64_t)shape->num_channels * num_frames;
    int32_t *d_pcm = NULL, *d_res = NULL, *d_prm = NULL; double *d_st = NULL;
    void *stage = NULL; int transient = 0;
    const uint64_t nb_a = align_up(nb), pb_a = align_up(pb);
    int ret = hstage_get(ctx, 2 * nb_a + pb_a + align_up(sb), &stage, &transient);
    if (ret != LNN_OK) return ret;
    d_pcm = (int32_t *)stage; d_res = (int32_t *)((uint8_t *)stage + nb_a); d_prm = (int32_t *)((uint8_t *)stage + 2 * nb_a); d_st = (double *)((uint8_t *)stage + 2 * nb_a + pb_a);
    ret = LNN_NG;
    if (hipMemcpyAsync(d_pcm, pcm, nb, hipMemcpyHostToDevice, ctx->stream) != hipSuccess) { snprintf(ctx->err, sizeof(ctx->err), "H2D failed"); goto done; }
    if (hipMemsetAsync(d_prm, 0, pb, ctx->stream) != hipSuccess || hipMemsetAsync(d_st, 0, sb, ctx->stream) != hipSuccess) { snprintf(ctx->err, sizeof(ctx->err), "memset failed"); goto done; }
    ret = LINNEAmd_EncodeFramesDevice(ctx, shape, d_pcm, num_samples, num_frames, d_res, d_prm, d_st);
    if (ret != LNN_OK) goto done;
    ret = LNN_NG;
    if (hipMemcpyAsync(residual, d_res, nb, hipMemcpyDeviceToHost, ctx->stream) != hipSuccess
            || hipMemcpyAsync(params, d_prm, pb, hipMemcpyDeviceToHost, ctx->stream) != hipSuccess
            || hipMemcpyAsync(stats, d_st, sb, hipMemcpyDeviceToHost, ctx->stream) != hipSuccess) { snprintf(ctx->err, sizeof(ctx->err), "D2H failed"); goto done; }
    {
        hipError_t e = hipStreamSynchronize(ctx->stream);
        if (e != hipSuccess) { snprintf(ctx->err, sizeof(ctx->err), "stream sync: %s", hipGetErrorString(e)); goto done; }
    }
    ret = LNN_OK;
done:
    if (ret != LNN_OK || transient) hipStreamSynchronize(ctx->stream);
    if (transient) hipFree(stage);
    return ret;
}

extern "C" int LINNEAmd_DecodeFramesHost(struct LINNEAmdContext *ctx, const struct LINNEAmdShape *shape,
        int32_t *data, const uint32_t *num_samples, uint32_t num_frames, const int32_t *params)
{
    if (!ctx) return LNN_INVALID_ARGUMENT;
    if (!shape || !data || !params) return LNN_INVALID_ARGUMENT;
    if (num_frames == 0) return LNN_OK;
    { HostShape hs_; int r_ = shape_info(shape, &hs_); if (r_ != LNN_OK) { snprintf(ctx->err, sizeof(ctx->err), "invalid shape"); return r_; }
      if ((r_ = params_in_range(ctx, &hs_, shape->num_channels, params, num_frames)) != LNN_OK) return r_; }
    HIPCHK(ctx, hipSetDevice(ctx->device));
    const uint64_t CS = (uint64_t)shape->num_channels * shape->num_samples_per_block;
    const uint64_t nb = sizeof(int32_t) * CS * num_frames, pb = sizeof(int32_t) * LINNE_AMD_PARAM_WORDS * (uint64_t)shape->num_channels * num_frames;
    int32_t *d_data = NULL, *d_prm = NULL;
    void *stage = NULL; int transient = 0;
    int ret = hstage_get(ctx, align_up(nb) + pb, &stage, &transient);
    if (ret != LNN_OK) return ret;
    d_data = (int32_t *)stage; d_prm = (int32_t *)((uint8_t *)stage + align_up(nb));
    ret = LNN_NG;
    if (hipMemcpyAsync(d_data, data, nb, hipMemcpyHostToDevice, ctx->stream) != hipSuccess
            || hipMemcpyAsync(d_prm, params, pb, hipMemcpyHostToDevice, ctx->stream) != hipSuccess) { snprintf(ctx->err, sizeof(ctx->err), "H2D failed"); goto done; }
    ret = LINNEAmd_DecodeFramesDevice(ctx, shape, d_data, num_samples, num_frames, d_prm);
    if (ret != LNN_OK) goto done;
    ret = LNN_NG;
    if (hipMemcpyAsync(data, d_data, nb, hipMemcpyDeviceToHost, ctx->stream) != hipSuccess) { snprintf(ctx->err, sizeof(ctx->err), "D2H failed"); goto done; }
    {
        hipError_t e = hipStreamSynchronize(ctx->stream);
        if (e != hipSuccess) { snprintf(ctx->err, sizeof(ctx->err), "stream sync: %s", hipGetErrorString(e)); goto done; }
    }
    ret = LNN_OK;
done:
    if (ret != LNN_OK || transient) hipStreamSynchronize(ctx->stream);
    if (transient) hipFree(stage);
    return ret;
}


extern "C" int LINNEAmd_RicePlanDevice(struct LINNEAmdContext *ctx, const struct LINNEAmdShape *shape,
        const int32_t *d_residual, const uint32_t *h_num_samples, uint32_t num_frames, uint8_t *d_plan)
{
    if (!ctx) return LNN_INVALID_ARGUMENT;
    ctx->err[0] = 0;
    if (!shape || !d_residual || !d_plan) { snprintf(ctx->err, sizeof(ctx->err), "null argument"); return LNN_INVALID_ARGUMENT; }
    if (num_frames == 0) return LNN_OK;
    HostShape hs;
    int ret = shape_info(shape, &hs);
    if (ret != LNN_OK) { snprintf(ctx->err, sizeof(ctx->err), "invalid shape"); return ret; }
    HIPCHK(ctx, hipSetDevice(ctx->device));
    if (ctx->rice_nsteps == 0) ctx->rice_nsteps = lnn_rice_k2_steps(ctx->rice_steps);
    int m;
    if ((ret = meta_acquire(ctx, num_frames, &m)) != LNN_OK) return ret;
    uint32_t *nsm = ctx->meta_h[m];
    if ((ret = copy_lengths(ctx, shape, h_num_samples, num_frames, nsm)) != LNN_OK) return ret;
    if ((ret = ensure_buf(ctx, (void **)&ctx->d_plan_nsmp, &ctx->plan_nsmp_cap, sizeof(uint32_t) * (uint64_t)num_frames)) != LNN_OK) return ret;
    HIPCHK(ctx, hipMemcpyAsync(ctx->d_plan_nsmp, nsm, sizeof(uint32_t) * num_frames, hipMemcpyHostToDevice, ctx->stream));
    HIPCHK(ctx, hipEventRecord(ctx->meta_ev[m], ctx->stream));
    ctx->meta_used[m] = 1;
    RicePlanArgs a; memset(&a, 0, sizeof(a));
    a.resid = d_residual; a.nsmp = ctx->d_plan_nsmp; a.plan = d_plan; a.C = shape->num_channels; a.S = shape->num_samples_per_block;
    a.nsteps = ctx->rice_nsteps;
    for (uint32_t i = 0; i < 32; i++) a.steps[i] = ctx->rice_steps[i];
    a.guard = ctx->rice_guard > 0.0 ? ctx->rice_guard : LNN_RICE_GUARD;
    const uint64_t CF = (uint64_t)num_frames * shape->num_channels;
    for (uint64_t c0 = 0; c0 < CF; ) {
        uint64_t cnt = CF - c0;
        const uint64_t lim = (0x7FFFFFFFull / a.C) * a.C;
        if (cnt > lim) cnt = lim;
        RicePlanArgs b = a;
        b.resid = d_residual + c0 * a.S; b.plan = d_plan + c0 * LINNE_AMD_RICE_PLAN_BYTES; b.nsmp = ctx->d_plan_nsmp + c0 / a.C;
        const int sp_ = span_begin(ctx, LINNE_AMD_T_RICE_PLAN, ctx->stream);
        if (b.S <= REMIT_LDS_SAMPLES) hipLaunchKernelGGL(k_rice_plan<true>, dim3((uint32_t)cnt), dim3(RICE_THREADS), sizeof(uint32_t) * (b.S + 1025u), ctx->stream, b);
        else hipLaunchKernelGGL(k_rice_plan<false>, dim3((uint32_t)cnt), dim3(RICE_THREADS), 0, ctx->stream, b);
        span_end(ctx, sp_, ctx->stream);
        c0 += cnt;
    }
    HIPCHK(ctx, hipGetLastError());
    return LNN_OK;
}

extern "C" int LINNEAmd_RiceEmitDevice(struct LINNEAmdContext *ctx, const struct LINNEAmdShape *shape,
        const int32_t *d_residual, uint32_t num_frames, const uint8_t *d_plan,
        uint32_t *d_offsets, uint8_t *d_packed, uint64_t packed_capacity)
{
    if (!ctx) return LNN_INVALID_ARGUMENT;
    ctx->err[0] = 0;
    if (!shape || !d_residual || !d_plan || !d_offsets || !d_packed) { snprintf(ctx->err, sizeof(ctx->err), "null argument"); return LNN_INVALID_ARGUMENT; }
    if (num_frames == 0) return LNN_OK;
    const uint64_t CF = (uint64_t)num_frames * shape->num_channels;
    if (CF > 0x7FFFFFFFull || ctx->plan_nsmp_cap < sizeof(uint32_t) * (uint64_t)num_frames) { snprintf(ctx->err, sizeof(ctx->err), "RiceEmitDevice: call RicePlanDevice for the same batch first"); return LNN_INVALID_ARGUMENT; }
    HIPCHK(ctx, hipSetDevice(ctx->device));
    RiceEmitArgs a; memset(&a, 0, sizeof(a));
    a.resid = d_residual; a.nsmp = ctx->d_plan_nsmp; a.plan = d_plan; a.offsets = d_offsets; a.packed = d_packed;
    a.packed_cap = packed_capacity & ~(uint64_t)15; a.C = shape->num_channels; a.S = shape->num_samples_per_block; a.CF = (uint32_t)CF;
    a.cap_bytes = shape->num_samples_per_block * 4u;
    { const char *e_ = getenv("LINNE_AMD_RICE_EMIT_CAP"); if (e_) a.cap_bytes = (uint32_t)atol(e_); }
    { const int sp_ = span_begin(ctx, LINNE_AMD_T_RICE_EMIT, ctx->stream);
      hipLaunchKernelGGL(k_rice_scan, dim3(1), dim3(RSCAN_THREADS), 0, ctx->stream, a);
      if (a.S <= REMIT_LDS_SAMPLES) hipLaunchKernelGGL(k_rice_emit<true>, dim3((uint32_t)CF), dim3(REMIT_THREADS), sizeof(uint32_t) * (a.S + REMIT_THREADS + 1u), ctx->stream, a);
      else hipLaunchKernelGGL(k_rice_emit<false>, dim3((uint32_t)CF), dim3(REMIT_THREADS), 0, ctx->stream, a);
      span_end(ctx, sp_, ctx->stream); }
    HIPCHK(ctx, hipGetLastError());
    return LNN_OK;
}

static int rice_decode_launch(LINNEAmdContext *ctx, hipStream_t st, const struct LINNEAmdShape *shape, const uint8_t *seg, uint64_t nbytes,
        const uint64_t *bitpos, const uint64_t *bitend, const uint32_t *nsmp, uint32_t F, int32_t *resid, uint64_t *endbit)
// ... 1591 lines not shown
    int first = -1;
    for (uint32_t i = 0; i < num_tracks; i++) {
        tracks[i].result = host[i].result;
        if (host[i].result == LNN_OK) tracks[i].parcor_state = host[i].state;
        else if (first < 0) first = (int)i;
    }
    if (first < 0) return LNN_OK;
    snprintf(ctx->err, sizeof(ctx->err), "track %d: %.*s", first, (int)sizeof(ctx->err) - 24, host[first].text);
    return host[first].result;
}


extern "C" int64_t LINNEAmd_GetLastSpliceCount(struct LINNEAmdContext *ctx, int which)
{
    if (!ctx || which < 0 || which > 5) return -1;
    return ctx->splice_count[which];
}

static int sp_ensure(LINNEAmdContext *ctx, void **ptr, uint64_t *cap, uint64_t need, bool pinned)
{
    if (*cap >= need) return LNN_OK;
    ctx->splice_count[5]++;
    HIPCHK(ctx, hipStreamSynchronize(ctx->stream));
    if (*ptr) HIPCHK(ctx, pinned ? hipHostFree(*ptr) : hipFree(*ptr));
    *ptr = NULL; *cap = 0;
    if (pinned) HIPCHK(ctx, hipHostMalloc(ptr, need, hipHostMallocDefault)); else HIPCHK(ctx, hipMalloc(ptr, need));
    *cap = need;
    return LNN_OK;
}

struct SpHost { char text[200]; };

static int sp_run(LINNEAmdContext *ctx, struct LINNEAmdSplice *splices, uint32_t N, uint32_t group_frames, std::vector<SpOutput> &outs, std::vector<SpHost> &host)
{
    std::vector<SpStream> streams;
    std::vector<const LINNEAmdStreamIndex *> sx;
    std::vector<SpCut> cuts;
    std::vector<const uint8_t *> cut_bytes;
    outs.resize(N); host.resize(N);
    for (uint32_t k = 0; k < N; k++) {
        const struct LINNEAmdSplice &s = splices[k];
        SpOutput &o = outs[k];
        memset(&o, 0, sizeof(o)); host[k].text[0] = 0;
        o.cut0 = (uint32_t)cuts.size(); o.ncuts = 0; o.capacity = s.capacity;
        o.why0 = (!s.d_out || (!s.cuts && s.num_cuts)) ? SP_WHY_NULL : (((uintptr_t)s.d_out & 3u) ? SP_WHY_ALIGN : SP_WHY_NONE);
        if (o.why0 || !s.num_cuts) continue;
        if ((uint64_t)cuts.size() + s.num_cuts > 0x7FFFFFFFull) { snprintf(ctx->err, sizeof(ctx->err), "SpliceStreamsDevice: too many cuts in one call"); return LNN_NG; }
        o.ncuts = s.num_cuts;
        for (uint32_t i = 0; i < s.num_cuts; i++) {
            const struct LINNEAmdCut &c = s.cuts[i];
            SpCut pc; pc.stream = -1; pc.first = c.first_sample; pc.n = c.num_samples;
            if (c.index && c.d_stream) {
                if (c.index->device != ctx->device) o.why0 = SP_WHY_DEVICE;
                size_t j = sx.size();
                while (j > 0 && sx[j - 1] != c.index) j--;
                if (j == 0) {
                    const LINNEAmdStreamIndex *x = c.index;
                    SpStream st;
                    st.off = x->h_off; st.first = x->h_first; st.size = x->h_size; st.nsmp = x->h_nsmp; st.nb = x->nb; st.num_samples = x->header.num_samples;
                    st.channels = x->header.num_channels; st.bits = x->header.bits_per_sample; st.rate = x->header.sampling_rate;
                    st.block = x->header.num_samples_per_block; st.preset = x->header.preset; st.ms = (uint32_t)x->header.ch_process_method;
                    st.fail_block = x->fail_block; st.fail_code = x->fail_code;
                    sx.push_back(x); streams.push_back(st); j = sx.size();
                }
                pc.stream = (int32_t)(j - 1);
            }
            cuts.push_back(pc); cut_bytes.push_back(c.d_stream);
        }
    }
    std::vector<SpPiece> pieces;
    sp_plan(streams.data(), cuts.data(), outs.data(), N, pieces);
    auto refuse = [&](uint32_t k, int code, const char *text) {
        outs[k].result = code; outs[k].copied_blocks = outs[k].encoded_blocks = 0; outs[k].bytes = 0;
        snprintf(host[k].text, sizeof(host[k].text), "%s", text);
    };
    for (uint32_t k = 0; k < N; k++) {
        const SpOutput &o = outs[k];
        if (o.result == LNN_OK) continue;
        if (o.result == LNN_INVALID_ARGUMENT && o.why) snprintf(host[k].text, sizeof(host[k].text), "SpliceStreamsDevice: %s", sp_why_text(o.why));
        else {
            const LINNEAmdStreamIndex *x = sx[cuts[o.cut0 + o.fail_cut].stream];
            snprintf(host[k].text, sizeof(host[k].text), "cut %u: block %lld (byte %llu of the stream): %s", o.fail_cut, (long long)x->fail_block, (unsigned long long)x->fail_off,
                    x->fail_code == LNN_NG ? "a block no encoder writes" : "damaged or truncated stream");
        }
    }
    HIPCHK(ctx, hipSetDevice(ctx->device));
    ctx->nspans = 0; ctx->outer_keep = 1;
    if (ctx->timing) (void)hipEventRecord(ctx->ev[0], ctx->stream);
    std::vector<uint32_t> frag;
    uint64_t runs_max = 0, live = 0;
    for (uint32_t k = 0; k < N; k++) if (outs[k].result == LNN_OK) { live++; runs_max += outs[k].npieces; }
    for (uint32_t i = 0; i < pieces.size(); i++) if (pieces[i].frag) frag.push_back(i);
    if (!live) return LNN_OK;
    const uint32_t nfrag = (uint32_t)frag.size();
    std::vector<uint64_t> o_pcm(nfrag), o_str(nfrag), room(nfrag);
    uint64_t at = 0;
    for (uint32_t f = 0; f < nfrag; f++) {
        const SpPiece &p = pieces[frag[f]];
        const SpStream &st = streams[cuts[outs[p.out].cut0 + p.cut].stream];
        o_pcm[f] = at; at = (at + sizeof(int32_t) * (uint64_t)st.channels * (p.b - p.a) + 15u) & ~(uint64_t)15u;
        room[f] = LINNE_HEADER_SIZE + 64u + (uint64_t)st.channels * st.block * 8u;
        o_str[f] = at; at = (at + room[f] + 15u) & ~(uint64_t)15u;
    }
    const uint64_t o_runs = at; at = align_up(at + sizeof(SpRun) * (runs_max + 1u));
    const uint64_t o_hptr = at; at = align_up(at + sizeof(uint8_t *) * live);
    const uint64_t o_hbytes = at; at = align_up(at + 32u * live);
    const uint64_t stage_bytes = at - o_runs;
    SX_TRY(sp_ensure(ctx, &ctx->spl, &ctx->spl_cap, at, false));
    SX_TRY(sp_ensure(ctx, &ctx->spl_stage, &ctx->spl_stage_cap, stage_bytes, true));
    uint8_t *sd = (uint8_t *)ctx->spl, *hs_ = (uint8_t *)ctx->spl_stage;
    if (nfrag) {
        std::vector<struct LINNEAmdWindow> win(nfrag);
        for (uint32_t f = 0; f < nfrag; f++) {
            const SpPiece &p = pieces[frag[f]];
            const uint32_t ci = outs[p.out].cut0 + p.cut;
            win[f].index = sx[cuts[ci].stream]; win[f].d_stream = cut_bytes[ci]; win[f].first_sample = p.a; win[f].num_samples = p.b - p.a;
            win[f].d_pcm = (int32_t *)(sd + o_pcm[f]); win[f].pcm_stride = p.b - p.a; win[f].result = LNN_OK;
        }
        int ret = LINNEAmd_DecodeWindowsDevice(ctx, win.data(), nfrag, group_frames);
        if (ret != LNN_OK && strncmp(ctx->err, "window ", 7) != 0) return LNN_NG;
        for (uint32_t f = 0; f < nfrag; f++) {
            const SpPiece &p = pieces[frag[f]];
            if (win[f].result != LNN_OK && outs[p.out].result == LNN_OK) {
                char text[sizeof(host[0].text)];
                snprintf(text, sizeof(text), "cut %u, samples [%llu, %llu): DecodeWindowsDevice -> %d (a block whose Rice codes do not end where its size field says)", p.cut,
                        (unsigned long long)p.a, (unsigned long long)p.b, win[f].result);
                refuse(p.out, win[f].result, text);
            }
        }
        std::vector<struct LINNEAmdTrack> trk;
        std::vector<uint32_t> trk_frag;
        for (uint32_t f = 0; f < nfrag; f++) {
            const SpPiece &p = pieces[frag[f]];
            if (outs[p.out].result != LNN_OK) continue;
            struct LINNEAmdTrack t; memset(&t, 0, sizeof(t));
            t.header = sx[cuts[outs[p.out].cut0 + p.cut].stream]->header; t.header.num_samples = (uint32_t)(p.b - p.a);
            t.d_pcm = (const int32_t *)(sd + o_pcm[f]); t.pcm_stride = p.b - p.a; t.d_out = sd + o_str[f]; t.capacity = room[f];
            t.parcor_state = 0.0;
            trk.push_back(t); trk_frag.push_back(f);
        }
        if (!trk.empty()) {
            ret = LINNEAmd_EncodeStreamsDevice(ctx, trk.data(), (uint32_t)trk.size(), group_frames);
            if (ret != LNN_OK && strncmp(ctx->err, "track ", 6) != 0) return LNN_NG;
            for (size_t j = 0; j < trk.size(); j++) {
                SpPiece &p = pieces[frag[trk_frag[j]]];
                if (trk[j].result == LNN_OK) { p.bytes = trk[j].out_bytes - LINNE_HEADER_SIZE; continue; }
                if (outs[p.out].result != LNN_OK) continue;
                char text[sizeof(host[0].text)];
                snprintf(text, sizeof(text), "cut %u, samples [%llu, %llu): EncodeStreamDevice refuses the edge block with %d", p.cut, (unsigned long long)p.a, (unsigned long long)p.b, trk[j].result);
                refuse(p.out, trk[j].result, text);
            }
        }
        ctx->err[0] = 0;
    }
    sp_place(outs.data(), N, pieces.data());
    SpRun *h_runs = (SpRun *)hs_;
    uint8_t **h_hptr = (uint8_t **)(hs_ + (o_hptr - o_runs));
    uint8_t *h_hbytes = hs_ + (o_hbytes - o_runs);
    uint32_t nruns = 0, nh = 0; uint64_t nchunks = 0;
    std::vector<uint32_t> frag_of(pieces.size(), 0u);
    for (uint32_t f = 0; f < nfrag; f++) frag_of[frag[f]] = f;
    for (uint32_t k = 0; k < N; k++) {
        SpOutput &o = outs[k];
        if (o.result == LNN_INSUFFICIENT_BUFFER) {
            snprintf(host[k].text, sizeof(host[k].text), "the stream takes %llu bytes, the buffer holds %llu", (unsigned long long)o.bytes, (unsigned long long)o.capacity);
            o.copied_blocks = o.encoded_blocks = 0;
        }
        if (o.result != LNN_OK) continue;
        struct LINNEHeader h = sx[cuts[o.cut0].stream]->header;
        h.num_samples = (uint32_t)o.total_samples;
        SX_TRY((int)LINNEEncoder_EncodeHeader(&h, h_hbytes + 32u * (uint64_t)nh, LINNE_HEADER_SIZE));
        h_hptr[nh++] = splices[k].d_out;
        for (uint32_t i = 0; i < o.npieces; i++) {
            const SpPiece &p = pieces[o.piece0 + i];
            if (!p.bytes) continue;
            SpRun &r = h_runs[nruns++];
            r.src = p.frag ? sd + o_str[frag_of[o.piece0 + i]] + LINNE_HEADER_SIZE : cut_bytes[o.cut0 + p.cut] + p.a;
            r.dst = splices[k].d_out + p.dst; r.n = p.bytes; r.chunk0 = nchunks;
            nchunks += sp_run_chunks((uint64_t)(uintptr_t)r.dst, r.n);
            ctx->splice_count[4] += (int64_t)p.bytes;
        }
        ctx->splice_count[0]++; ctx->splice_count[1] += o.copied_blocks; ctx->splice_count[2] += o.encoded_blocks;
    }
    ctx->splice_count[3] = nruns;
    if (nh) {
        memset(&h_runs[nruns], 0, sizeof(SpRun)); h_runs[nruns].chunk0 = nchunks;
        HIPCHK(ctx, hipMemcpyAsync(sd + o_runs, hs_, stage_bytes, hipMemcpyHostToDevice, ctx->stream));
        if (nruns) {
            const uint32_t grid = nchunks < SP_MAX_GRID ? (uint32_t)nchunks : SP_MAX_GRID;
            SX_LAUNCH(LINNE_AMD_SPLICE_T_COPY, k_sp_copy, dim3(grid), dim3(SP_THREADS), 0, ctx->stream, (const SpRun *)(sd + o_runs), nruns, nchunks);
        }
        SX_LAUNCH(LINNE_AMD_SPLICE_T_HEADER, k_sb_header, dim3((nh * 32u + 255u) / 256u), dim3(256), 0, ctx->stream, (uint8_t *const *)(sd + o_hptr), (const uint8_t *)(sd + o_hbytes), nh);
    }
    return LNN_OK;
}

extern "C" int LINNEAmd_SpliceStreamsDevice(struct LINNEAmdContext *ctx, struct LINNEAmdSplice *splices, uint32_t num_splices, uint32_t group_frames)
{
    if (!ctx) return LNN_INVALID_ARGUMENT;
    ctx->err[0] = 0;
    for (int i = 0; i < 6; i++) ctx->splice_count[i] = 0;
    if (num_splices == 0) return LNN_OK;
    if (!splices) { snprintf(ctx->err, sizeof(ctx->err), "SpliceStreamsDevice: null argument"); return LNN_INVALID_ARGUMENT; }
    std::vector<SpOutput> outs;
    std::vector<SpHost> host;
    int ret;
    try { ret = sp_run(ctx, splices, num_splices, group_frames, outs, host); }
    catch (const std::bad_alloc &) { snprintf(ctx->err, sizeof(ctx->err), "out of host memory"); ret = LNN_NG; }
    const bool began = ctx->outer_keep != 0;
    ctx->outer_keep = 0; ctx->span_keep = 0;
    if (began && ctx->timing) { (void)hipEventRecord(ctx->ev[1], ctx->stream); ctx->ev_valid = 1; }
    if (began) {
        ctx->splice_count[5]++;
        if (hipStreamSynchronize(ctx->stream) != hipSuccess && ret == LNN_OK) { snprintf(ctx->err, sizeof(ctx->err), "SpliceStreamsDevice: hipStreamSynchronize failed"); ret = LNN_NG; }
    }
    if (ret != LNN_OK) {
        if (!ctx->err[0]) snprintf(ctx->err, sizeof(ctx->err), "SpliceStreamsDevice: failed with %d", ret);
        for (uint32_t i = 0; i < num_splices; i++) { splices[i].result = LNN_NG; splices[i].out_bytes = 0; splices[i].copied_blocks = splices[i].encoded_blocks = 0; }
        for (int i = 0; i < 5; i++) ctx->splice_count[i] = 0;
        return LNN_NG;
    }
    int first = -1;
    for (uint32_t i = 0; i < num_splices; i++) {
        const SpOutput &o = outs[i];
        splices[i].result = o.result;
        splices[i].out_bytes = (o.result == LNN_OK || o.result == LNN_INSUFFICIENT_BUFFER) ? o.bytes : 0u;
        splices[i].copied_blocks = o.result == LNN_OK ? o.copied_blocks : 0u;
        splices[i].encoded_blocks = o.result == LNN_OK ? o.encoded_blocks : 0u;
        if (o.result != LNN_OK && first < 0) first = (int)i;
    }
    if (first < 0) return LNN_OK;
    snprintf(ctx->err, sizeof(ctx->err), "splice %d: %.*s", first, (int)sizeof(ctx->err) - 24, host[first].text);
    return outs[first].result;
}

extern "C" int64_t lnn_splice_plan(const uint64_t *stream_rec, const uint64_t *const *tabs, uint32_t nstreams, const uint64_t *cut_rec, uint32_t ncuts,
        const uint64_t *out_in, uint32_t nouts, const uint64_t *frag_bytes, uint32_t nfrag_bytes, uint64_t *out_rec, uint64_t *piece_rec, uint64_t piece_cap)
{
    try {
        std::vector<SpStream> streams(nstreams);
        std::vector<std::vector<uint32_t>> narrow(2 * (size_t)nstreams);
        for (uint32_t s = 0; s < nstreams; s++) {
            const uint64_t *r = stream_rec + 10u * (uint64_t)s;
            SpStream &st = streams[s];
            st.nb = (uint32_t)r[0]; st.num_samples = r[1]; st.channels = (uint32_t)r[2]; st.bits = (uint32_t)r[3]; st.rate = (uint32_t)r[4]; st.block = (uint32_t)r[5];
            st.preset = (uint32_t)r[6]; st.ms = (uint32_t)r[7]; st.fail_block = (int64_t)r[8]; st.fail_code = (int32_t)r[9];
            st.off = tabs[4u * s]; st.first = tabs[4u * s + 1u];
            for (int w = 0; w < 2; w++) { std::vector<uint32_t> &v = narrow[2u * s + w]; v.resize(st.nb); for (uint32_t i = 0; i < st.nb; i++) v[i] = (uint32_t)tabs[4u * s + 2u + w][i]; }
            st.size = narrow[2u * s].data(); st.nsmp = narrow[2u * s + 1u].data();
        }
        std::vector<SpCut> cuts(ncuts);
        for (uint32_t i = 0; i < ncuts; i++) { cuts[i].stream = (int32_t)(int64_t)cut_rec[3u * i]; cuts[i].first = cut_rec[3u * i + 1u]; cuts[i].n = cut_rec[3u * i + 2u]; }
        std::vector<SpOutput> outs(nouts);
        for (uint32_t k = 0; k < nouts; k++) { memset(&outs[k], 0, sizeof(SpOutput)); outs[k].cut0 = (uint32_t)out_in[4u * k]; outs[k].ncuts = (uint32_t)out_in[4u * k + 1u]; outs[k].capacity = out_in[4u * k + 2u]; outs[k].why0 = (int)out_in[4u * k + 3u]; }
        std::vector<SpPiece> pieces;
        sp_plan(streams.data(), cuts.data(), outs.data(), nouts, pieces);
        uint32_t f = 0;
        for (SpPiece &p : pieces) if (p.frag) { p.bytes = f < nfrag_bytes ? frag_bytes[f] : 0u; f++; }
        sp_place(outs.data(), nouts, pieces.data());
        for (uint32_t k = 0; k < nouts; k++) {
            const SpOutput &o = outs[k]; uint64_t *r = out_rec + 8u * (uint64_t)k;
            r[0] = (uint64_t)(int64_t)o.result; r[1] = (uint64_t)o.why; r[2] = o.bytes; r[3] = o.total_samples; r[4] = o.copied_blocks; r[5] = o.encoded_blocks; r[6] = o.piece0; r[7] = o.npieces;
        }
        for (size_t i = 0; i < pieces.size() && i < piece_cap; i++) {
            const SpPiece &p = pieces[i]; uint64_t *r = piece_rec + 8u * i;
            r[0] = p.out; r[1] = p.cut; r[2] = p.frag; r[3] = p.blocks; r[4] = p.a; r[5] = p.b; r[6] = p.bytes; r[7] = p.dst;
        }
        return (int64_t)pieces.size();
    } catch (const std::bad_alloc &) { return -1; }
}


#define LNN_Q_HEADER 48
#define LNN_Q_CHUNK 16
#define LNN_Q_LAYER 24
extern "C" int64_t lnn_forms_query(int mode, const struct LINNEAmdShape *shape, const uint32_t *num_samples, uint32_t num_frames,
        uint64_t arena_bytes, int ctx_streams, int has_side, uint32_t af_iters, uint32_t learning, int data_aligned, int64_t *out, uint64_t cap)
{
    HostShape hs;
    if (!out || num_frames == 0 || shape_info(shape, &hs) != LNN_OK) return -1;
    LnnKnobs knob; memset(&knob, 0, sizeof(knob));
    lnn_knobs_read_context(&knob); lnn_knobs_read_call(&knob);
    const uint32_t C = shape->num_channels, S = shape->num_samples_per_block;
    uint64_t n = 0;
    uint32_t *meta = NULL; LnnClassTable *tab = NULL;
#define PUT(v) do { if (n >= cap) { free(meta); free(tab); return -1; } out[n++] = (int64_t)(v); } while (0)
    if (mode == 1) {
        LnnDecodeForms df;
        lnn_decode_forms(&hs, C, S, shape->ch_process_method, num_frames, data_aligned != 0, SP_LDS_BYTES(S) <= LEV_LDS_BUDGET, &knob, &df);
        PUT(df.call); PUT(df.ms_separate);
        for (uint32_t l = 0; l < hs.L; l++) { const LnnDecLayer &d = df.layer[l]; PUT(d.form); PUT(d.nch); PUT(d.pb); PUT(d.de); PUT(d.ms_fold); }
        return (int64_t)n;
    }
    int forced = 0;
    if (ctx_streams < 0) ctx_streams = lnn_context_streams(&forced);
    meta = (uint32_t *)malloc(sizeof(uint32_t) * 3 * (size_t)num_frames);
    tab = (LnnClassTable *)calloc(1, sizeof(LnnClassTable));
    LnnCallClasses cc;
    if (!meta || !tab || lnn_call_classes(tab, shape, &hs, &knob, num_samples, num_frames, meta, meta + num_frames, meta + 2 * (size_t)num_frames, &cc) != LNN_CLS_OK) { free(meta); free(tab); return -1; }
    const uint64_t per_frame = frame_scratch_bytes(shape, &hs, af_iters, learning);
    if (arena_bytes == 0) arena_bytes = 6ull << 30;
    if (arena_bytes < per_frame * 4 + 65536) arena_bytes = per_frame * 4 + 65536;
    const LnnSplit sp = lnn_call_split(arena_bytes, per_frame, num_frames, C, hs.R, ctx_streams, forced != 0, &knob);
    PUT(cc.branch); PUT(cc.nlen); PUT(cc.na_max); PUT(cc.prod_ok); PUT(sp.nsub); PUT(sp.use_sub); PUT(sp.chunk); PUT(sp.part_bytes);
    PUT((num_frames + sp.chunk - 1) / sp.chunk); PUT(lnn_stats_rows_form(&knob, num_frames, C, S, hs.P[0])); PUT(per_frame); PUT(hs.L);
    PUT(sp.streams_forced); PUT(0); PUT(0); PUT(0);
    for (uint32_t i = 0; i < LNN_MAXCLS; i++) PUT(i < cc.nlen ? cc.lens[i] : 0);
    for (uint32_t i = 0; i < LNN_MAXCLS; i++) PUT(i < cc.nlen ? cc.slot_of[i] : 0);
    for (uint32_t f0 = 0; f0 < num_frames; f0 += (uint32_t)sp.chunk) {
        const uint32_t Fc = (num_frames - f0 < sp.chunk) ? (num_frames - f0) : (uint32_t)sp.chunk;
        for (int fin = 0; fin < (af_iters ? 2 : 1); fin++) {
            const LnnChunkIn in = { &hs, C, S, Fc, tab->cls, meta + f0, &knob, sp.use_sub, has_side != 0, af_iters, learning, fin != 0 };
            LnnChunkForms cf;
            lnn_chunk_forms(&in, &cf);
            RowRuns rr; lnn_build_runs(&rr, meta + f0, Fc, C * hs.R);
            PUT(f0); PUT(Fc); PUT((uint64_t)Fc * C * (fin ? 1u : hs.R)); PUT(fin); PUT(cf.fwd_loss_on); PUT(cf.fuse_cfg); PUT(cf.fuse_all); PUT(cf.last_layer_all);
            PUT(cf.prep_defer); PUT(cf.hist); PUT(cf.chain_sum); PUT(cf.chain_sum_wave); PUT(cf.cascade_walk); PUT(rr.mixed); PUT(rr.n); PUT(cf.present);
            for (uint32_t l = 0; l < hs.L; l++) {
                const LnnLayerForms &lf = cf.layer[l];
                uint32_t nleft = 0, left_first = 0, left_frames = 0;
                if (lf.long_any && !lf.long_all && !lf.fir_small)
                    for (uint32_t f = 0, g = 0; lnn_next_left_run(&lf, meta + f0, Fc, g, &f, &g); nleft++) { if (!nleft) left_first = f; left_frames += g - f; }
                PUT(lf.fir_spec); PUT(lf.hist_layer); PUT(lf.hist_all); PUT(lf.beside); PUT(lf.lev_wave); PUT(lf.nlev); PUT(lf.nlev ? lf.lev[0].ride : 0); PUT(lf.last_layer);
                PUT(lf.long_any); PUT(lf.long_all); PUT(lf.search_form); PUT(lf.fir_small); PUT(lf.sel_wave); PUT(lf.fwd_loss); PUT(lf.fwd_loss_mw); PUT(lf.forward);
                PUT(lf.forward_walk); PUT(nleft); PUT(left_first); PUT(left_frames); PUT(lf.long_mask); PUT(lf.lev_beside); PUT(lf.lev_carrier); PUT(lf.lev_carrier < lf.nlev ? lf.lev[lf.lev_carrier].ride : LNN_MAXT);
            }
        }
    }
    free(meta); free(tab);
    return (int64_t)n;
#undef PUT
}

extern "C" int64_t lnn_classes_replay(const struct LINNEAmdShape *shapes, const uint32_t *lengths, const uint32_t *counts, uint32_t num_calls, int64_t *out, uint64_t cap)
{
    if (!shapes || !lengths || !counts || !out || cap < (uint64_t)num_calls * (2 + LNN_MAXCLS)) return -1;
    LnnKnobs knob; memset(&knob, 0, sizeof(knob));
    lnn_knobs_read_context(&knob); lnn_knobs_read_call(&knob);
    LnnClassTable *tab = (LnnClassTable *)calloc(1, sizeof(LnnClassTable));
    if (!tab) return -1;
    uint64_t n = 0;
    for (uint32_t i = 0; i < num_calls; i++) {
        HostShape hs; LnnCallClasses cc;
        uint32_t *meta = (uint32_t *)malloc(sizeof(uint32_t) * 3 * (size_t)(counts[i] ? counts[i] : 1));
        const bool ok = meta && shape_info(&shapes[i], &hs) == LNN_OK
                && lnn_call_classes(tab, &shapes[i], &hs, &knob, lengths, counts[i], meta, meta + counts[i], meta + 2 * (size_t)counts[i], &cc) == LNN_CLS_OK;
        free(meta);
        if (!ok) { free(tab); return -1; }
        out[n++] = cc.branch; out[n++] = tab->ncls;
        for (uint32_t s = 0; s < LNN_MAXCLS; s++) out[n++] = s < tab->ncls ? tab->cls[s].n : 0;
        lengths += counts[i];
    }
    free(tab);
    return (int64_t)n;
}
```

linne_amd/csrc/lnn_forms.h:

```cpp
#ifndef LNN_FORMS_H_INCLUDED
#define LNN_FORMS_H_INCLUDED

#include <math.h>
#include <stdint.h>
#include <stdlib.h>
#include <string.h>

#include "linne_amd.h"

#if defined(__HIPCC__)
#define LNN_HD __host__ __device__ __forceinline__
#else
#define LNN_HD inline
#endif

#define LNN_MAXT        8
#define LNN_MAXU        128
#define LNN_MAXP        128
#define LNN_MAXL        3
#define LNN_MAXR        4
#define LNN_MAXCLS      16
#define LNN_MAXCH       8
#define LNN_ACW         256
#define LNN_MAXSUB      8
#define LNN_META        8
#define LNN_FIR_TILE 2048u
#define LNN_FIR_WAVES   4u
#define LNN_SELW_MAXPART 64u
#define LNN_SEARCH_JOB_MIN 8u
#define LNN_LEV_MAXRIDE 3u
#define LEV_LDS(np_) (sizeof(double) * 64 * (size_t)(2 * (np_) + 3))
#define LEV_LDS_BUDGET ((size_t)160 * 1024)
#define LNN_SUB_TILE_SMALL 16u
#define LNN_SUB_SMALL_LDS ((size_t)8 * (2 * LNN_SUB_TILE_SMALL * 65 + 2 * LNN_MAXT * 32))
#define LNN_LEV_BESIDE_MIN 32768u
#define LNN_LEV_BESIDE_DEFAULT 1

struct DevClass {
    uint32_t n;
    uint32_t na;
    uint32_t sin_off;
    uint32_t pad;
    uint32_t ntrials[LNN_MAXL];
    uint32_t trial_u[LNN_MAXL][LNN_MAXT];
    double   trial_div[LNN_MAXL][LNN_MAXT];
    uint32_t wt_off[LNN_MAXL][LNN_MAXT];
};

#define LNN_MAXRUN LNN_MAXCLS
struct RowRuns { uint32_t n; uint32_t mixed; uint32_t row_begin[LNN_MAXRUN + 1]; uint32_t blk_begin[LNN_MAXRUN + 1]; };

struct HostShape { uint32_t L, R, P[LNN_MAXL], coef_off[LNN_MAXL], maxP; double regs[LNN_MAXR]; };

struct LnnPlanView { uint32_t L, S, hist, search_long, fused_last, P[LNN_MAXL]; };

template <class PlanT> LNN_HD bool search_long_takes(const PlanT &p, uint32_t layer, const DevClass &c)
{
    const uint32_t P = p.P[layer];
    uint32_t nt = 0; for (uint32_t u = 1; u <= P && u <= (uint32_t)LNN_MAXU; u <<= 1) nt++;
    return p.search_long && layer > 0 && layer + 1 < p.L && (P == 128u || P == 64u) && c.ntrials[layer] == nt && (c.na % LNN_FIR_TILE) == 0;
}

template <class PlanT> LNN_HD bool fwd_loss_takes(const PlanT &p, uint32_t layer, uint32_t na) { return p.fused_last && layer + 1 == p.L && (na % (4u * p.P[layer])) == 0; }

template <class PlanT> LNN_HD bool hist_takes(const PlanT &p, uint32_t layer, const DevClass &c)
{
    const uint32_t P = p.P[layer];
    uint32_t nt = 0; for (uint32_t u = 1; u <= P && u <= (uint32_t)LNN_MAXU; u <<= 1) nt++;
    return p.hist && P >= 64u && c.ntrials[layer] == nt && (c.na % (16u << (nt - 1))) == 0 && (c.na >> (nt - 1)) >= 32u && (p.S & 3u) == 0;
}
static inline uint32_t lnn_all_trials(uint32_t P) { uint32_t nt = 0; for (uint32_t u = 1; u <= P && u <= (uint32_t)LNN_MAXU; u <<= 1) nt++; return nt; }

struct LnnKnobs {
    int fwd_loss;
    int lev_ride;
    int lev_beside;
    int lev_wave;
    int search_two;
    int search_job;
    int fir_small;
    int fir_spec;
    int force_exact;
    int sort, l0_products, wide, search_long, rows16, prep_general;
    int stats_rows;
    int hist;
    int decode_kernel;
    int rows8;
    int streams;
    int nostats;
    int fwd_loss_mw;
    int prep_defer;
    int last_layer;
    int decode_fused;
    uint32_t dbg_maxtr;
};
static inline int lnn_env_int(const char *name, int dflt) { const char *e = getenv(name); return e ? atoi(e) : dflt; }
static inline void lnn_knobs_read_context(LnnKnobs *k)
{
    k->force_exact = lnn_env_int("LINNE_AMD_EXACT", 0);
    k->fir_spec = lnn_env_int("LINNE_AMD_SPECULATE", 1);
    k->lev_ride = lnn_env_int("LINNE_AMD_LEV_RIDE", 1);
    k->lev_wave = lnn_env_int("LINNE_AMD_LEV_WAVE", 1);
    k->lev_beside = lnn_env_int("LINNE_AMD_LEV_BESIDE", -1);
    k->search_two = lnn_env_int("LINNE_AMD_SEARCH_TWO", 1);
    k->search_job = lnn_env_int("LINNE_AMD_SEARCH_JOB", -1);
    k->fwd_loss = lnn_env_int("LINNE_AMD_FWD_LOSS", -1);
    k->fir_small = lnn_env_int("LINNE_AMD_FIR_SMALL", 1);
}
static inline void lnn_knobs_read_call(LnnKnobs *k)
{
    k->sort = lnn_env_int("LINNE_AMD_SORT", 1);
    k->l0_products = lnn_env_int("LINNE_AMD_L0_PRODUCTS", 1);
    k->wide = lnn_env_int("LINNE_AMD_WIDE", 1);
    k->search_long = lnn_env_int("LINNE_AMD_SEARCH_LONG", 1);
    k->rows16 = lnn_env_int("LINNE_AMD_ROWS16", 1);
    k->prep_general = lnn_env_int("LINNE_AMD_PREP_GENERAL", 0);
    k->prep_defer = lnn_env_int("LINNE_AMD_PREP_DEFER", 1);
    k->fwd_loss_mw = lnn_env_int("LINNE_AMD_FWD_LOSS_MW", 1);
    k->last_layer = lnn_env_int("LINNE_AMD_LAST_LAYER", 1);
    k->stats_rows = lnn_env_int("LINNE_AMD_STATS_ROWS", -1);
    { const char *e = getenv("LINNE_AMD_HIST"); k->hist = e ? (atoi(e) != 0) : -1; }
    k->rows8 = lnn_env_int("LINNE_AMD_DECODE_ROWS8", -1);
    k->decode_fused = lnn_env_int("LINNE_AMD_DECODE_FUSED", 1);
    { const char *e = getenv("LINNE_AMD_DECODE_KERNEL"); k->decode_kernel = !e ? 0 : (strcmp(e, "wave") == 0 ? 1 : (strcmp(e, "pipe") == 0 ? 3 : (strcmp(e, "rows") == 0 ? 4 : 2))); }
    k->streams = lnn_env_int("LINNE_AMD_STREAMS", 0);
    if (k->streams < 0) k->streams = 0;
#ifdef LNN_TIMING_EXPERIMENTS
    k->dbg_maxtr = (uint32_t)lnn_env_int("LINNE_AMD_DBG_MAXTR", 0);
    k->nostats = lnn_env_int("LINNE_AMD_DBG_NOSTATS", 0);
#else
    k->dbg_maxtr = 0; k->nostats = 0;
#endif
}

static inline int lnn_context_streams(int *forced)
{
    const char *env = getenv("LINNE_AMD_STREAMS");
    int ns = env ? atoi(env) : 2;
    *forced = env != NULL;
    if (ns < 1) ns = 1;
    if (ns > LNN_MAXSUB) ns = LNN_MAXSUB;
    return ns >= 2 ? ns : 0;
}

static inline double lnn_welch_div(uint32_t unit_samples) { return 4.0 * pow((double)(unit_samples - 1u), -2.0); }

static inline void lnn_make_class(const HostShape *hs, uint32_t S, uint32_t n, uint64_t *sin_total, uint64_t *wt_total, DevClass *out)
{
    DevClass c; memset(&c, 0, sizeof(c));
    c.n = n;
    uint32_t na = ((n + 7u) / 8u) * 8u;
    if (na < hs->maxP) na = hs->maxP;
    if (na > S) na = S;
    c.na = na;
    c.sin_off = (uint32_t)*sin_total; *sin_total += n;
    for (uint32_t l = 0; l < hs->L; l++) {
        const uint32_t maxu = hs->P[l] < 128u ? hs->P[l] : 128u;
        uint32_t nt = 0;
        for (uint32_t u = 1; u <= maxu; u <<= 1) {
            if ((hs->P[l] % u) != 0 || (na % u) != 0) continue;
            c.trial_u[l][nt] = u;
            c.trial_div[l][nt] = lnn_welch_div(na / u);
            c.wt_off[l][nt] = (uint32_t)*wt_total;
            { const uint32_t pu = hs->P[l] / u; *wt_total += na / u + (pu > 4 ? pu : 4); *wt_total = (*wt_total + 3u) & ~(uint64_t)3u; }
            nt++;
        }
        c.ntrials[l] = nt;
    }
    *out = c;
}

struct LnnClassTable { DevClass cls[LNN_MAXCLS]; struct LINNEAmdShape shape; int valid; uint32_t ncls; uint64_t sin_total, wt_total; };
enum { LNN_CLS_FIRST = 0, LNN_CLS_REUSE = 1, LNN_CLS_APPEND = 2, LNN_CLS_RESTART_SHAPE = 3, LNN_CLS_RESTART_OVERFLOW = 4 };
enum { LNN_CLS_OK = 0, LNN_CLS_BAD_LENGTH = 1, LNN_CLS_TOO_MANY = 2 };
struct LnnCallClasses {
    int error; uint32_t error_frame;
    int branch;
    uint32_t nlen, lens[LNN_MAXCLS], slot_of[LNN_MAXCLS];
    uint32_t na_max;
    int prod_ok;
};

static inline int lnn_call_classes(LnnClassTable *tab, const struct LINNEAmdShape *shape, const HostShape *hs, const LnnKnobs *k,
        const uint32_t *h_num_samples, uint32_t F, uint32_t *idx, uint32_t *map, uint32_t *raw, LnnCallClasses *out)
{
    const uint32_t S = shape->num_samples_per_block;
    uint32_t *lens = out->lens, *slot_of = out->slot_of, nlen = 0;
    memset(out, 0, sizeof(*out));
    {
        uint32_t last_n = 0, last_k = 0;
        for (uint32_t f = 0; f < F; f++) {
            const uint32_t n = h_num_samples ? h_num_samples[f] : S;
            if (n == 0 || n > S) { out->error_frame = f; return out->error = LNN_CLS_BAD_LENGTH; }
            uint32_t kk = last_k;
            if (n != last_n || nlen == 0) {
                for (kk = 0; kk < nlen; kk++) if (lens[kk] == n) break;
                if (kk == nlen) {
                    if (nlen == LNN_MAXCLS) return out->error = LNN_CLS_TOO_MANY;
                    lens[nlen++] = n;
                }
                last_n = n; last_k = kk;
            }
            raw[f] = kk;
        }
    }
    out->nlen = nlen;
    const bool same_shape = tab->valid && memcmp(&tab->shape, shape, sizeof(*shape)) == 0;
    uint32_t missing = 0;
    for (uint32_t kk = 0; kk < nlen; kk++) {
        uint32_t j = 0;
        if (same_shape) for (; j < tab->ncls; j++) if (tab->cls[j].n == lens[kk]) break;
        slot_of[kk] = (same_shape && j < tab->ncls) ? j : 0xFFFFFFFFu;
        if (slot_of[kk] == 0xFFFFFFFFu) missing++;
    }
    out->branch = LNN_CLS_REUSE;
    if (missing) {
        out->branch = LNN_CLS_APPEND;
        if (!same_shape || tab->ncls + missing > LNN_MAXCLS) {
            out->branch = same_shape ? LNN_CLS_RESTART_OVERFLOW : (tab->valid ? LNN_CLS_RESTART_SHAPE : LNN_CLS_FIRST);
            tab->ncls = 0; tab->sin_total = 0; tab->wt_total = 0;
            memset(tab->cls, 0, sizeof(tab->cls));
            for (uint32_t kk = 0; kk < nlen; kk++) slot_of[kk] = 0xFFFFFFFFu;
        }
        for (uint32_t kk = 0; kk < nlen; kk++) if (slot_of[kk] == 0xFFFFFFFFu) {
            lnn_make_class(hs, S, lens[kk], &tab->sin_total, &tab->wt_total, &tab->cls[tab->ncls]);
            slot_of[kk] = tab->ncls++;
        }
        tab->shape = *shape; tab->valid = 1;
    }
    for (uint32_t kk = 0; kk < nlen; kk++) if (tab->cls[slot_of[kk]].na > out->na_max) out->na_max = tab->cls[slot_of[kk]].na;
    if (k->sort == 0) { for (uint32_t f = 0; f < F; f++) { idx[f] = slot_of[raw[f]]; map[f] = f; } }
    else {
        uint32_t count[LNN_MAXCLS + 1];
        memset(count, 0, sizeof(count));
        for (uint32_t f = 0; f < F; f++) count[raw[f] + 1]++;
        for (uint32_t kk = 0; kk < nlen; kk++) count[kk + 1] += count[kk];
        for (uint32_t f = 0; f < F; f++) { const uint32_t pos = count[raw[f]]++; idx[pos] = slot_of[raw[f]]; map[pos] = f; }
    }
    for (uint32_t l = 0; l < hs->L; l++) {
        if (hs->P[l] > 16u || !k->l0_products) continue;
        uint32_t nt = 0; for (uint32_t u = 1; u <= hs->P[l]; u <<= 1) nt++;
        int ok = 1;
        for (uint32_t kk = 0; kk < nlen; kk++) { const DevClass &c = tab->cls[slot_of[kk]]; if (c.ntrials[l] != nt || (c.na % (1u << nt)) != 0) ok = 0; }
        if (ok) out->prod_ok |= 1 << l;
    }
    for (uint32_t l = 0; l < hs->L; l++) {
        if (hs->P[l] < 32u || hs->P[l] > 128u || !k->wide || (uint64_t)F * shape->num_channels * (l == 0 ? 1u : hs->R) > 64u) continue;
        int ok = 1;
        for (uint32_t kk = 0; kk < nlen; kk++) { const DevClass &c = tab->cls[slot_of[kk]]; if (c.ntrials[l] == 0 || (c.na % (1u << c.ntrials[l])) != 0) ok = 0; }
        if (ok) out->prod_ok |= 1 << l;
    }
    return LNN_CLS_OK;
}

static inline void lnn_build_runs(RowRuns *rr, const uint32_t *idx, uint32_t F, uint32_t rpf)
{
    uint32_t n = 0, f = 0;
    rr->row_begin[0] = 0; rr->blk_begin[0] = 0;
    while (f < F) {
        uint32_t g = f + 1;
        while (g < F && idx[g] == idx[f]) g++;
        if (n == LNN_MAXRUN) { n = 0; break; }
        rr->row_begin[n + 1] = g * rpf;
        rr->blk_begin[n + 1] = rr->blk_begin[n] + ((g - f) * rpf + 63u) / 64u;
        n++; f = g;
    }
    rr->mixed = 0;
    if (n == 0) { n = 1; rr->mixed = 1; rr->row_begin[1] = F * rpf; rr->blk_begin[1] = (F * rpf + 63u) / 64u; }
    rr->n = n;
}

struct LnnSplit { uint32_t nsub; uint64_t part_bytes, chunk; bool streams_forced, use_sub; };
static inline LnnSplit lnn_call_split(uint64_t arena_bytes, uint64_t per_frame, uint32_t num_frames, uint32_t C, uint32_t R,
        int ctx_nsub, bool ctx_forced, const LnnKnobs *k)
{
    LnnSplit s;
    uint32_t nsub = ctx_nsub > 0 ? (uint32_t)ctx_nsub : 1u;
    s.streams_forced = ctx_forced || k->streams > 0;
    if (k->streams > 0 && (uint32_t)k->streams < nsub) nsub = (uint32_t)k->streams;
    while (nsub > 1 && ((arena_bytes - 65536) / nsub < per_frame * 2 || num_frames < nsub * 512u)) nsub--;
    if (!s.streams_forced) while (nsub > 1 && (uint64_t)(num_frames / nsub) * C * R < 32768u) nsub--;
    s.nsub = nsub;
    s.part_bytes = ((arena_bytes - 65536) / nsub) & ~(uint64_t)255;
    uint64_t chunk = s.part_bytes / per_frame;
    if (chunk == 0) chunk = 1;
    {
        const uint64_t even = (num_frames + nsub - 1) / nsub;
        if (chunk > even) chunk = even;
        const uint64_t lim = 4194304u / ((uint64_t)C * R);
        if (chunk > lim) chunk = lim;
        uint64_t nchunks = (num_frames + chunk - 1) / chunk;
        nchunks = ((nchunks + nsub - 1) / nsub) * nsub;
        chunk = (num_frames + nchunks - 1) / nchunks;
    }
    s.chunk = chunk;
    s.use_sub = ctx_nsub > 0 && (nsub > 1 || (s.streams_forced && k->streams != 1));
    return s;
}

static inline bool lnn_stats_rows_form(const LnnKnobs *k, uint32_t num_frames, uint32_t C, uint32_t S, uint32_t P0)
{
    const bool rows_form = k->stats_rows >= 0 ? (k->stats_rows != 0) : ((uint64_t)num_frames * C >= 1024u);
    return rows_form && (S & 3u) == 0 && (P0 == 2u || P0 == 4u);
}

struct LnnLevLaunch { uint32_t t, u, threads, ride; size_t lds; };
struct LnnLayerForms {
    bool fir_spec;
    bool hist_layer, hist_all;
    bool beside;
    bool lev_wave;
    bool lev_inline;
    bool lev_beside;
    uint32_t lev_carrier;
    uint32_t nlev; LnnLevLaunch lev[LNN_MAXT];
    bool last_layer;
    bool long_any, long_all;
    uint32_t long_mask;
    int search_form;
    bool fir_small;
    bool sel_wave;
    bool fwd_loss, fwd_loss_mw;
    bool forward, forward_walk;
};
struct LnnChunkForms {
    bool fwd_loss_on, fuse_cfg, fuse_all, last_layer_all, prep_defer, hist;
    uint32_t present;
    bool chain_sum, chain_sum_wave;
    bool cascade_walk;
    LnnLayerForms layer[LNN_MAXL];
};
struct LnnChunkIn {
    const HostShape *hs; uint32_t C, S, Fc;
    const DevClass *cls; const uint32_t *idx;
    const LnnKnobs *k; bool use_sub, has_side; uint32_t af_iters, learning;
    bool final_pass;
};

static inline void lnn_chunk_forms(const LnnChunkIn *in, LnnChunkForms *cf)
{
    const HostShape &hs = *in->hs; const LnnKnobs &k = *in->k;
    const uint32_t S = in->S, Fc = in->Fc, L = hs.L, Plast = hs.P[L - 1];
    const bool fin = in->final_pass;
    const uint64_t CF = (uint64_t)Fc * in->C, J = CF * (fin ? 1u : hs.R);
    memset(cf, 0, sizeof(*cf));
    for (uint32_t f = 0; f < Fc; f++) cf->present |= 1u << in->idx[f];
    LnnPlanView pv; memset(&pv, 0, sizeof(pv));
    pv.L = L; pv.S = S; pv.hist = 1; pv.fused_last = 1; pv.search_long = k.search_long ? 1u : 0u;
    for (uint32_t l = 0; l < L; l++) pv.P[l] = hs.P[l];
    uint32_t fwd_mask = 0, lastnt_mask = 0, hist_mask[LNN_MAXL] = { 0, 0, 0 }, long_mask[LNN_MAXL] = { 0, 0, 0 };
    for (uint32_t s = 0; s < LNN_MAXCLS; s++) if ((cf->present >> s) & 1u) {
        const DevClass &c = in->cls[s];
        if (fwd_loss_takes(pv, L - 1, c.na)) fwd_mask |= 1u << s;
        if (c.ntrials[L - 1] == lnn_all_trials(Plast)) lastnt_mask |= 1u << s;
        for (uint32_t l = 0; l < L; l++) {
            if (hist_takes(pv, l, c)) hist_mask[l] |= 1u << s;
            if (search_long_takes(pv, l, c)) long_mask[l] |= 1u << s;
        }
    }
    cf->fwd_loss_on = !fin && ((k.fwd_loss < 0) ? (J >= 24576u) : (k.fwd_loss != 0));
    cf->fuse_cfg = cf->fwd_loss_on && L > 1 && (Plast == 2u || Plast == 4u || Plast == 8u || Plast == 16u);
    cf->fuse_all = cf->fuse_cfg && (cf->present & ~fwd_mask) == 0;
    cf->last_layer_all = cf->fuse_all && k.last_layer && !k.force_exact && !in->af_iters && !in->learning
            && (J >= (in->use_sub ? 49152u : 81920u) || (k.last_layer == 2 && J > 256u)) && (cf->present & ~lastnt_mask) == 0;
    cf->prep_defer = k.prep_defer && !k.prep_general && (S & 3u) == 0 && CF * S * sizeof(int32_t) <= 0xFFFFFFFFull;
    RowRuns rr; lnn_build_runs(&rr, in->idx, Fc, in->C * hs.R);
    cf->hist = !fin && (k.hist >= 0 ? (k.hist != 0) : (J >= 12288u));
    if (rr.mixed) cf->hist = false;
    const uint32_t tiles = (S + LNN_FIR_TILE - 1) / LNN_FIR_TILE;
    for (uint32_t l = 0; l < L; l++) {
        LnnLayerForms &lf = cf->layer[l];
        const uint32_t P = hs.P[l], maxu = P < 128u ? P : 128u;
        const bool last = l + 1 == L;
        lf.fir_spec = !fin && k.fir_spec && !last;
        lf.hist_layer = cf->hist && P >= 64u;
        lf.hist_all = cf->hist && (cf->present & ~hist_mask[l]) == 0;
        lf.beside = lf.hist_layer && !lf.hist_all && in->has_side;
        lf.lev_wave = J <= 64u && k.lev_wave;
        lf.lev_carrier = LNN_MAXT;
        if (!lf.lev_wave) {
            uint32_t ride = LNN_MAXT;
            for (uint32_t t = 1, u = 2; u <= maxu && k.lev_ride; u <<= 1, t++)
                if (LEV_LDS(P) + LNN_LEV_MAXRIDE * LEV_LDS(P / u) <= LEV_LDS_BUDGET) { ride = t; break; }
            const bool beside_size = k.lev_beside >= 0 ? (k.lev_beside != 0) : (LNN_LEV_BESIDE_DEFAULT && J >= LNN_LEV_BESIDE_MIN);
            lf.lev_beside = beside_size && lf.hist_layer && P == 128u && in->has_side && ride >= 2u && ride < LNN_MAXT
                    && LEV_LDS(P / 2u) + LNN_LEV_MAXRIDE * LEV_LDS(P >> ride) <= LEV_LDS_BUDGET && LEV_LDS(P) + LNN_SUB_SMALL_LDS <= LEV_LDS_BUDGET;
            lf.lev_inline = lf.lev_beside && k.lev_beside == 2;
            if (ride < LNN_MAXT) lf.lev_carrier = lf.lev_beside ? 1u : 0u;
            for (uint32_t t = 0, u = 1; u <= maxu && t < (ride < LNN_MAXT ? ride : LNN_MAXT); u <<= 1, t++) {
                const bool carry = (t == lf.lev_carrier);
                LnnLevLaunch &v = lf.lev[lf.nlev++];
                v.t = t; v.u = u;
                v.lds = LEV_LDS(P / u) + (carry ? LNN_LEV_MAXRIDE * LEV_LDS(P >> ride) : 0);
                v.threads = carry ? 64 * (1 + LNN_LEV_MAXRIDE) : 64;
                v.ride = carry ? ride : (uint32_t)LNN_MAXT;
            }
        }
        lf.last_layer = cf->last_layer_all && last;
        if (!lf.last_layer) {
            lf.long_mask = (lf.fir_spec && !fin) ? long_mask[l] : 0u;
            lf.long_any = (cf->present & lf.long_mask) != 0;
            lf.long_all = (cf->present & ~lf.long_mask) == 0;
            const bool per_job = k.search_two && (k.search_job < 0 ? J >= LNN_SEARCH_JOB_MIN : k.search_job != 0);
            lf.search_form = per_job ? 2 : (k.search_two ? 1 : 0);
            lf.fir_small = P <= 16u && k.fir_small;
            lf.sel_wave = J <= 256u && (uint64_t)tiles * LNN_FIR_WAVES <= LNN_SELW_MAXPART;
            lf.fwd_loss = last && cf->fuse_cfg;
            lf.fwd_loss_mw = lf.fwd_loss && J < 65536u && k.fwd_loss_mw;
        }
        lf.forward = !(fin && last) && !(last && cf->fuse_all);
        lf.forward_walk = lf.forward && lf.fir_spec && J >= 4096u;
    }
    cf->chain_sum = !fin && !cf->fuse_all;
    cf->chain_sum_wave = cf->chain_sum && J <= 1024u;
    cf->cascade_walk = CF >= 1024u;
}

static inline bool lnn_next_left_run(const LnnLayerForms *lf, const uint32_t *idx, uint32_t Fc, uint32_t from, uint32_t *f, uint32_t *g)
{
    uint32_t a = from;
    while (a < Fc && ((lf->long_mask >> idx[a]) & 1u)) a++;
    if (a >= Fc) return false;
    uint32_t b = a + 1;
    while (b < Fc && !((lf->long_mask >> idx[b]) & 1u)) b++;
    *f = a; *g = b;
    return true;
}

enum { LNN_DEC_LAYERS = 0, LNN_DEC_WAVE = 1, LNN_DEC_PIPE = 2 };
enum { LNN_DL_FUSED_L0 = 0, LNN_DL_ROWS = 1, LNN_DL_ROWS8 = 2, LNN_DL_SMALL = 3, LNN_DL_BIG = 4, LNN_DL_GENERAL = 5 };
struct LnnDecLayer {
    int form;
    int nch;
    uint32_t pb;
    bool de;
    bool ms_fold;
};
struct LnnDecodeForms { int call; LnnDecLayer layer[LNN_MAXL]; bool ms_separate; };
static inline void lnn_decode_forms(const HostShape *hs, uint32_t C, uint32_t S, uint32_t ms, uint32_t num_frames, bool rows_ptr_ok, bool pipe_fits,
        const LnnKnobs *k, LnnDecodeForms *df)
{
    memset(df, 0, sizeof(*df));
    const uint32_t CF = num_frames * C;
    const bool rows_fit = (S & 3u) == 0u && rows_ptr_ok;
    const int form = k->decode_kernel ? k->decode_kernel : (CF < (rows_fit ? 1536u : 6144u) ? 3 : 0);
    const bool ms_foldable = ms && C >= 2u && C <= 64u && (C & (C - 1u)) == 0u;
    df->ms_separate = ms != 0;
    if (form == 3 && pipe_fits) { df->call = LNN_DEC_PIPE; return; }
    if (form == 1 || form == 3) { df->call = LNN_DEC_WAVE; return; }
    df->call = LNN_DEC_LAYERS;
    for (uint32_t l = 0; l < hs->L; l++) {
        LnnDecLayer &d = df->layer[l];
        const uint32_t P = hs->P[l];
        d.de = (l == 0);
        d.nch = P <= 16u ? 0 : (P == 32u ? 1 : (P == 64u ? 3 : (P == 128u ? 7 : -1)));
        if (d.de && d.nch == 0 && form != 2 && rows_fit && P <= 4u && k->decode_fused) {
            d.form = LNN_DL_FUSED_L0; d.ms_fold = ms_foldable;
        } else if (d.nch >= 0 && form != 2 && rows_fit) {
            d.form = LNN_DL_ROWS; d.pb = (d.nch == 0 && P <= 4u) ? 4u : 0u;
            if (d.nch == 0 && (k->rows8 < 0 ? CF >= 20480u : k->rows8 != 0)) { d.form = LNN_DL_ROWS8; d.pb = P <= 4u ? 4u : (P <= 8u ? 8u : 16u); }
            d.ms_fold = d.de && ms_foldable;
        } else {
            d.pb = P;
            d.form = (P == 2u || P == 4u || P == 8u || P == 16u) ? LNN_DL_SMALL : ((P == 32u || P == 64u || P == 128u) ? LNN_DL_BIG : LNN_DL_GENERAL);
        }
        if (d.ms_fold) df->ms_separate = false;
    }
}
#endif
```

linne_amd/csrc/lnn_k_levinson.h:

```cpp
#ifndef LNN_K_LEVINSON_H_INCLUDED
#define LNN_K_LEVINSON_H_INCLUDED

__device__ __forceinline__ void levinson_problem(const Plan &p, uint32_t layer, uint32_t t, uint32_t unit, double *lev_lds, uint32_t lane, uint32_t job0)
{
    uint32_t job = job0 + lane;
    const bool inrange = job < p.J;
    if (!inrange) job = p.J - 1;
    const DevClass &c = job_class(p, job);
    const uint32_t P = p.P[layer], u = 1u << t, np = P >> t, P0 = p.P[0];
    const bool have = inrange && t < c.ntrials[layer];
    const uint32_t n = c.na / u;
    double *sa = lev_lds + lane, *sr = lev_lds + (size_t)(np + 2) * 64 + lane;
    const double reg = p.job_reg ? p.job_reg[job] : p.regs[job % p.R];
    const uint32_t ajob = (layer == 0) ? job - job % p.R : job;
    const double *r = p.acorr + ((size_t)ajob * LNN_MAXT + t) * LNN_ACW + (size_t)unit * (np + 1);
    double *h = p.tcoef + ((size_t)job * LNN_MAXT + t) * LNN_MAXP + (size_t)unit * np;
    const bool last = (layer + 1 == p.L);
    for (uint32_t i = 0; i <= np; i++) sr[(size_t)i * 64] = have ? r[i] : 0.0;
    for (uint32_t i = 0; i < np + 2; i++) sa[(size_t)i * 64] = 0.0;
    double tail = 0.0; int tail_set = 0;
    const double r0 = sr[0] * (1.0 + reg);
    const bool zero = (n < np) || (fabs(r0) < (double)FLT_EPSILON);
    {
        const double r1 = sr[64];
        double ek = r0;
        const double a1 = -r1 / r0;
        ek += r1 * a1;
        sa[0] = 1.0; sa[64] = a1;
        for (uint32_t k = 1; k < np; k++) {
            double gamma = 0.0;
            {
                const double *pa = sa, *pr = sr + (size_t)(k + 1) * 64;
                uint32_t i = 0;
                for (; i + 8 <= k + 1; i += 8) {
                    const double a0 = pa[0], a1_ = pa[64], a2 = pa[128], a3 = pa[192], a4 = pa[256], a5 = pa[320], a6 = pa[384], a7 = pa[448];
                    const double q0 = pr[0], q1 = *(pr - 64), q2 = *(pr - 128), q3 = *(pr - 192), q4 = *(pr - 256), q5 = *(pr - 320), q6 = *(pr - 384), q7 = *(pr - 448);
                    const double m0 = a0 * q0, m1 = a1_ * q1, m2 = a2 * q2, m3 = a3 * q3, m4 = a4 * q4, m5 = a5 * q5, m6 = a6 * q6, m7 = a7 * q7;
                    gamma += m0; gamma += m1; gamma += m2; gamma += m3; gamma += m4; gamma += m5; gamma += m6; gamma += m7;
                    pa += 512; pr -= 512;
                }
                for (; i + 4 <= k + 1; i += 4) {
                    const double a0 = pa[0], a1_ = pa[64], a2 = pa[128], a3 = pa[192];
                    const double q0 = pr[0], q1 = *(pr - 64), q2 = *(pr - 128), q3 = *(pr - 192);
                    gamma += a0 * q0; gamma += a1_ * q1; gamma += a2 * q2; gamma += a3 * q3;
                    pa += 256; pr -= 256;
                }
                for (; i <= k; i++) { gamma += pa[0] * pr[0]; pa += 64; pr -= 64; }
            }
            gamma /= -ek;
            ek *= (1.0 - gamma * gamma);
            const double a0n = 1.0 + gamma * 0.0;
            const double ak1 = 0.0 + gamma * 1.0;
            uint32_t i = 1, j = k;
            while (i + 6 < j) {
                double *pi = sa + (size_t)i * 64, *pj = sa + (size_t)j * 64;
                const double ai0 = pi[0], ai1 = pi[64], ai2 = pi[128], ai3 = pi[192];
                const double aj0 = pj[0], aj1 = *(pj - 64), aj2 = *(pj - 128), aj3 = *(pj - 192);
                pi[0] = ai0 + gamma * aj0;   pj[0] = aj0 + gamma * ai0;
                pi[64] = ai1 + gamma * aj1;  *(pj - 64) = aj1 + gamma * ai1;
                pi[128] = ai2 + gamma * aj2; *(pj - 128) = aj2 + gamma * ai2;
                pi[192] = ai3 + gamma * aj3; *(pj - 192) = aj3 + gamma * ai3;
                i += 4; j -= 4;
            }
            while (i < j) {
                const double ai = sa[(size_t)i * 64], aj = sa[(size_t)j * 64];
                sa[(size_t)i * 64] = ai + gamma * aj;
                sa[(size_t)j * 64] = aj + gamma * ai;
                i++; j--;
            }
            if (i == j) { const double ai = sa[(size_t)i * 64]; sa[(size_t)i * 64] = ai + gamma * ai; }
            sa[0] = a0n; sa[(size_t)(k + 1) * 64] = ak1;
            if (last && k == P0) { tail = -gamma; tail_set = 1; }
        }
    }
    if (!have) return;
    if (zero) {
        for (uint32_t k = 0; k < np; k++) h[k] = 0.0;
        tail = 0.0; tail_set = (np >= P0) ? 1 : 0;
    } else {
        for (uint32_t k = 0; k < np; k++) h[k] = sa[(size_t)(np - k) * 64];
        if (!(last && np > P0)) { tail = 0.0; tail_set = 0; }
    }
    if (last) {
        p.ptail[((size_t)job * LNN_MAXT + t) * LNN_MAXU + unit] = tail;
        p.ptail_set[((size_t)job * LNN_MAXT + t) * LNN_MAXU + unit] = (uint8_t)tail_set;
    }
}

#define LEV_MAXRIDE 3
__global__ __launch_bounds__(64 * (1 + LEV_MAXRIDE)) void k_levinson_lds(Plan p, uint32_t layer, uint32_t t, uint32_t ride)
{
    extern __shared__ __attribute__((aligned(16))) double lev_lds[];
    const uint32_t wave = threadIdx.x >> 6, lane = threadIdx.x & 63u, job0 = blockIdx.x * 64;
    if (wave == 0) { levinson_problem(p, layer, t, blockIdx.y, lev_lds, lane, job0); return; }
    const uint32_t nride = (blockDim.x >> 6) - 1u, nseat = nride * gridDim.y, seat = blockIdx.y * nride + (wave - 1u);
    double *mine = lev_lds + (size_t)(2 * (p.P[layer] >> t) + 3) * 64 + (size_t)(wave - 1u) * (2 * (p.P[layer] >> ride) + 3) * 64;
    const uint32_t maxu = p.P[layer] < (uint32_t)LNN_MAXU ? p.P[layer] : (uint32_t)LNN_MAXU;
    uint32_t q = 0;
    for (uint32_t tt = ride, u = 1u << ride; u <= maxu; tt++, u <<= 1)
        for (uint32_t unit = 0; unit < u; unit++, q++)
            if (q % nseat == seat) levinson_problem(p, layer, tt, unit, mine, lane, job0);
}

__global__ __launch_bounds__(64) void k_levinson_wave(Plan p, uint32_t layer)
{
    __shared__ __attribute__((aligned(16))) double sa[2][LNN_MAXP + 2], sr[LNN_MAXP + 2], sprod[LNN_MAXP + 2];
    const uint32_t job = blockIdx.x, lane = threadIdx.x;
    const uint32_t t = 31u - (uint32_t)__clz((int)(blockIdx.y + 1u)), unit = blockIdx.y + 1u - (1u << t);
    const DevClass &c = job_class(p, job);
    if (t >= c.ntrials[layer]) return;
    const uint32_t P = p.P[layer], u = 1u << t, np = P >> t, P0 = p.P[0];
    const uint32_t n = c.na / u;
    const double reg = p.job_reg ? p.job_reg[job] : p.regs[job % p.R];
    const uint32_t ajob = (layer == 0) ? job - job % p.R : job;
    const double *r = p.acorr + ((size_t)ajob * LNN_MAXT + t) * LNN_ACW + (size_t)unit * (np + 1);
    double *h = p.tcoef + ((size_t)job * LNN_MAXT + t) * LNN_MAXP + (size_t)unit * np;
    const bool last = (layer + 1 == p.L);
    for (uint32_t i = lane; i <= np; i += 64u) sr[i] = r[i];
    for (uint32_t i = lane; i < np + 2u; i += 64u) { sa[0][i] = 0.0; sa[1][i] = 0.0; }
    __builtin_amdgcn_wave_barrier();
    double tail = 0.0; int tail_set = 0;
    const double r0 = sr[0] * (1.0 + reg);
    const bool zero = (n < np) || (fabs(r0) < (double)FLT_EPSILON);
    uint32_t cur = 0;
    if (!zero) {
        const double r1 = sr[1];
        double ek = r0;
        const double a1 = -r1 / r0;
        ek += r1 * a1;
        if (lane == 0) { sa[0][0] = 1.0; sa[0][1] = a1; }
        __builtin_amdgcn_wave_barrier();
        for (uint32_t k = 1; k < np; k++) {
            const double *a = sa[cur];
            double *an = sa[cur ^ 1u];
            for (uint32_t i = lane; i <= k; i += 64u) sprod[i] = a[i] * sr[k + 1u - i];
            __builtin_amdgcn_wave_barrier();
            double gamma = 0.0;
            {
                uint32_t i = 0;
                for (; i + 8u <= k + 1u; i += 8u) {
                    const lnn_d2 m0 = *(const lnn_d2 *)(sprod + i), m1 = *(const lnn_d2 *)(sprod + i + 2), m2 = *(const lnn_d2 *)(sprod + i + 4), m3 = *(const lnn_d2 *)(sprod + i + 6);
                    gamma += m0.x; gamma += m0.y; gamma += m1.x; gamma += m1.y; gamma += m2.x; gamma += m2.y; gamma += m3.x; gamma += m3.y;
                }
                for (; i <= k; i++) gamma += sprod[i];
            }
            gamma /= -ek;
            ek *= (1.0 - gamma * gamma);
            for (uint32_t i = lane; i <= k + 1u; i += 64u) {
                double v;
                if (i == 0u) v = 1.0 + gamma * 0.0;
                else if (i == k + 1u) v = 0.0 + gamma * 1.0;
                else v = a[i] + gamma * a[k + 1u - i];
                an[i] = v;
            }
            __builtin_amdgcn_wave_barrier();
            cur ^= 1u;
            if (last && k == P0) { tail = -gamma; tail_set = 1; }
        }
    }
    if (zero) {
        for (uint32_t k = lane; k < np; k += 64u) h[k] = 0.0;
        tail = 0.0; tail_set = (np >= P0) ? 1 : 0;
    } else {
        for (uint32_t k = lane; k < np; k += 64u) h[k] = sa[cur][np - k];
        if (!(last && np > P0)) { tail = 0.0; tail_set = 0; }
    }
    if (last && lane == 0) {
        p.ptail[((size_t)job * LNN_MAXT + t) * LNN_MAXU + unit] = tail;
        p.ptail_set[((size_t)job * LNN_MAXT + t) * LNN_MAXU + unit] = (uint8_t)tail_set;
    }
}

#endif
```

Before: 223,000 frames/s.

## Stream Levinson autocorrelation from global scratch to shrink LDS footprint

New measurement: 222,900 frames/s. No clear change (-0.1%).

```diff
diff --git a/linne_amd/csrc/lnn_dev_common.h b/linne_amd/csrc/lnn_dev_common.h
--- a/linne_amd/csrc/lnn_dev_common.h
+++ b/linne_amd/csrc/lnn_dev_common.h
@@ -35,6 +35,7 @@
     double *acorr;
     double *tcoef;
     double *ptail; uint8_t *ptail_set;
+    double *lev_scr;
     double *tloss;
     double *tsum;
     uint32_t npart;
diff --git a/linne_amd/csrc/lnn_device.hip b/linne_amd/csrc/lnn_device.hip
--- a/linne_amd/csrc/lnn_device.hip
+++ b/linne_amd/csrc/lnn_device.hip
@@ -58,6 +58,7 @@
     hipEvent_t fork_ev[LNN_MAXSUB], join_ev[LNN_MAXSUB], lev_fork_ev[LNN_MAXSUB], lev_join_ev[LNN_MAXSUB];
     DevClass *d_cls; double *d_sin; uint64_t sin_cap; double *d_wt; uint64_t wt_cap; uint32_t *d_clsidx; uint64_t clsidx_cap; uint32_t *d_map;    uint32_t *d_nsmp; uint64_t nsmp_cap;
     LnnClassTable tab;
+    int last_lev_scratch;
     int last_search_form;
     const uint32_t *cur_idx;
     uint32_t *meta_h[LNN_META]; uint64_t meta_cap[LNN_META]; hipEvent_t meta_ev[LNN_META]; int meta_used[LNN_META]; int meta_next;
@@ -161,8 +162,9 @@
     ctx->arena_bytes = scratch_bytes;
     if ((e = hipMalloc((void **)&ctx->d_cls, sizeof(DevClass) * LNN_MAXCLS)) != hipSuccess) { CC_FAIL("hipMalloc(classes)"); hipFree(ctx->arena); hipStreamDestroy(ctx->stream); free(ctx); return NULL; }
     if ((e = hipMalloc((void **)&ctx->d_ucount, 4 * sizeof(uint32_t))) != hipSuccess) { CC_FAIL("hipMalloc(counter)"); }
-    lnn_knobs_read_context(&ctx->knob); ctx->last_search_form = -1;
+    lnn_knobs_read_context(&ctx->knob); ctx->last_search_form = -1; ctx->last_lev_scratch = -1;
     (void)hipFuncSetAttribute((const void *)k_levinson_lds, hipFuncAttributeMaxDynamicSharedMemorySize, (int)LEV_LDS_BUDGET);
+    (void)hipFuncSetAttribute((const void *)k_levinson_scr, hipFuncAttributeMaxDynamicSharedMemorySize, (int)LEV_LDS_BUDGET);
     (void)hipFuncSetAttribute((const void *)k_synth_pipe, hipFuncAttributeMaxDynamicSharedMemorySize, (int)LEV_LDS_BUDGET);
     if ((e = hipEventCreate(&ctx->ev[0])) != hipSuccess || (e = hipEventCreate(&ctx->ev[1])) != hipSuccess) { CC_FAIL("hipEventCreate"); }
 #undef CC_FAIL
@@ -331,6 +333,7 @@
     return cnt ? sum : -1.0;
 }
 extern "C" int LINNEAmd_GetLastSearchLongForm(struct LINNEAmdContext *ctx) { return ctx ? ctx->last_search_form : -1; }
+extern "C" int lnn_last_lev_scratch(struct LINNEAmdContext *ctx) { return ctx ? ctx->last_lev_scratch : -1; }
 extern "C" int LINNEAmd_GetLastTimingLaunches(struct LINNEAmdContext *ctx, int which)
 {
     if (!ctx) return 0;
@@ -545,7 +548,7 @@
 struct EncodeCall {
     const struct LINNEAmdShape *shape; HostShape hs; uint32_t C, S, num_frames, pcm16;
     const int32_t *d_pcm; int32_t *d_residual, *d_params; double *d_stats;
-    LnnSplit split;
+    LnnSplit split; uint64_t per_frame;
 };
 struct Chunk {
     LINNEAmdContext *ctx; hipStream_t st; const HostShape *hs;
@@ -554,6 +557,7 @@
     const uint32_t *idx;
     Plan p; LnnChunkForms forms;
     uint8_t *abase; uint64_t part_bytes;
+    uint64_t lev_room;
     uint32_t *af_best; double *af_loss, *af_reg; TrainArgs tr;
 };
 struct Pass {
@@ -601,7 +605,8 @@
     k.CF = (uint64_t)k.Fc * e.C; k.J = k.CF * e.hs.R;
     k.idx = ctx->cur_idx + f0;
     const uint64_t CF = k.CF, J = k.J;
-    const LnnChunkIn in = { &e.hs, e.C, S, k.Fc, ctx->tab.cls, k.idx, &ctx->knob, e.split.use_sub, ctx->has_side != 0, ctx->af_iters, ctx->learning, false };
+    k.lev_room = lnn_lev_room(e.split.part_bytes, e.per_frame, k.Fc);
+    const LnnChunkIn in = { &e.hs, e.C, S, k.Fc, ctx->tab.cls, k.idx, &ctx->knob, e.split.use_sub, ctx->has_side != 0, ctx->af_iters, ctx->learning, false, k.lev_room };
     lnn_chunk_forms(&in, &k.forms);
     Plan &p = k.p;
     fill_plan(p, e, k.Fc);
@@ -643,6 +648,7 @@
         TAKE(p.af_obj, double, CF * LNN_MAXU); TAKE(p.af_prev, double, CF * LNN_MAXU); TAKE(p.af_state, uint32_t, CF * LNN_MAXU);
         TAKE(p.af_prob, uint32_t, CF * LNN_MAXU); TAKE(p.af_nprob, uint32_t, 64); TAKE(p.af_pivot, double, CF * LNN_MAXU);
     }
+    for (uint32_t l = 0; l < e.hs.L; l++) if (k.forms.layer[l].lev_scratch && !p.lev_scr) TAKE(p.lev_scr, double, LNN_LEV_SCRATCH_BYTES(J, e.hs.P[l]) / sizeof(double));
 #undef TAKE
     if ((uint64_t)(a - k.abase) > k.part_bytes) { snprintf(ctx->err, sizeof(ctx->err), "internal: arena overflow"); return LNN_NG; }
     return LNN_OK;
@@ -667,6 +673,15 @@
         if (hipStreamCreateWithFlags(&ctx->sib[1], hipStreamNonBlocking) != hipSuccess) { (void)hipGetLastError(); ctx->sib[1] = ctx->side; }
     }
     k.sib = ctx->sib[k.slot & 1u];
+}
+
+static void launch_levinson_lds(LINNEAmdContext *ctx, hipStream_t st, const Plan &q, uint32_t l, uint32_t J, const LnnLevLaunch &v)
+{
+    const dim3 grid((J + 63) / 64, v.u), blk(v.threads);
+    if (v.t == 0 && q.P[l] >= 128u) ctx->last_lev_scratch = v.scratch ? 1 : 0;
+    if (!v.scratch) hipLaunchKernelGGL(k_levinson_lds, grid, blk, v.lds, st, q, l, v.t, v.ride);
+    else if (q.lev_scr) hipLaunchKernelGGL(k_levinson_scr, grid, blk, v.lds, st, q, l, v.t, v.ride);
+    else snprintf(ctx->err, sizeof(ctx->err), "internal: k_levinson_scr without its scratch");
 }
 
 static int launch_lags(Chunk &k, const Pass &ps, uint32_t l)
@@ -682,13 +697,13 @@
     if (lf.hist_layer) {
         for (int w = 0; w < 3; w++) {
             if (P == 64u && w == 1) continue;
-            const int sp_ = span_begin(ctx, LINNE_AMD_T_HIST_P + w, st); (void)launch_autocorr_hist(st, q, l, ps.cur, w, w == 2 && lf.lev_beside); span_end(ctx, sp_, st);
+            const int sp_ = span_begin(ctx, LINNE_AMD_T_HIST_P + w, st); (void)launch_autocorr_hist(st, q, l, ps.cur, w, w == 2 && lf.sub_small); span_end(ctx, sp_, st);
             if (w == 0 && lf.lev_beside) {
                 const LnnLevLaunch &v = lf.lev[0];
                 const hipStream_t ls = lf.lev_inline ? st : k.sib;
                 if (lf.lev_inline && lf.beside) HIPCHK(ctx, hipStreamWaitEvent(st, ctx->join_ev[k.slot], 0));
                 if (!lf.lev_inline) { HIPCHK(ctx, hipEventRecord(ctx->lev_fork_ev[k.slot], st)); HIPCHK(ctx, hipStreamWaitEvent(k.sib, ctx->lev_fork_ev[k.slot], 0)); }
-                hipLaunchKernelGGL(k_levinson_lds, dim3((ps.J + 63) / 64, v.u), dim3(v.threads), v.lds, ls, q, l, v.t, v.ride);
+                launch_levinson_lds(ctx, ls, q, l, ps.J, v);
                 if (!lf.lev_inline) HIPCHK(ctx, hipEventRecord(ctx->lev_join_ev[k.slot], k.sib));
             }
         }
@@ -709,7 +724,7 @@
     if (lf.lev_wave) hipLaunchKernelGGL(k_levinson_wave, dim3(ps.J, 2u * maxu - 1u), dim3(64), 0, st, q, l);
     else for (uint32_t i = lf.lev_beside ? 1u : 0u; i < lf.nlev; i++) {
         const LnnLevLaunch &v = lf.lev[i];
-        hipLaunchKernelGGL(k_levinson_lds, dim3((ps.J + 63) / 64, v.u), dim3(v.threads), v.lds, st, q, l, v.t, v.ride);
+        launch_levinson_lds(ctx, st, q, l, ps.J, v);
     }
     span_end(ctx, sp_, st);
 }
@@ -862,7 +877,7 @@
     lnn_build_runs(&q.runs[1], k.idx, k.Fc, k.C);
     q.job_reg = k.af_reg; q.af_best = k.af_best; q.af_loss = k.af_loss;
     hipLaunchKernelGGL(k_af_best, dim3((CF + 255) / 256), dim3(256), 0, st, p, k.af_best, k.af_loss, k.af_reg);
-    const LnnChunkIn in = { k.hs, k.C, k.S, k.Fc, ctx->tab.cls, k.idx, &ctx->knob, false, ctx->has_side != 0, ctx->af_iters, ctx->learning, true };
+    const LnnChunkIn in = { k.hs, k.C, k.S, k.Fc, ctx->tab.cls, k.idx, &ctx->knob, false, ctx->has_side != 0, ctx->af_iters, ctx->learning, true, k.lev_room };
     LnnChunkForms ff;
     lnn_chunk_forms(&in, &ff);
     Pass fp = { &q, &ff, CF, ctx->af_iters, 0 };
@@ -937,10 +952,11 @@
         HIPCHK(ctx, hipMalloc(&ctx->arena, per_frame * 4 + 65536));
         ctx->arena_bytes = per_frame * 4 + 65536;
     }
+    e.per_frame = per_frame;
     e.split = lnn_call_split(ctx->arena_bytes, per_frame, num_frames, e.C, e.hs.R, ctx->nsub, ctx->nsub_forced != 0, &ctx->knob);
     const LnnSplit &sp = e.split;
     if (!ctx->span_keep) ctx->nspans = 0;
-    ctx->last_search_form = -1;
+    ctx->last_search_form = -1; ctx->last_lev_scratch = -1;
     ctx->capture_n = 0;
     if (ctx->capture_on) {
         const uint64_t nrec = (uint64_t)num_frames * e.C * e.hs.R * e.hs.L * LNN_MAXT;
@@ -3138,17 +3154,29 @@
     if (arena_bytes == 0) arena_bytes = 6ull << 30;
     if (arena_bytes < per_frame * 4 + 65536) arena_bytes = per_frame * 4 + 65536;
     const LnnSplit sp = lnn_call_split(arena_bytes, per_frame, num_frames, C, hs.R, ctx_streams, forced != 0, &knob);
+    if (mode == 2) { PUT((num_frames + sp.chunk - 1) / sp.chunk); PUT(hs.L); PUT(per_frame); PUT(sp.part_bytes); }
+    else {
     PUT(cc.branch); PUT(cc.nlen); PUT(cc.na_max); PUT(cc.prod_ok); PUT(sp.nsub); PUT(sp.use_sub); PUT(sp.chunk); PUT(sp.part_bytes);
     PUT((num_frames + sp.chunk - 1) / sp.chunk); PUT(lnn_stats_rows_form(&knob, num_frames, C, S, hs.P[0])); PUT(per_frame); PUT(hs.L);
     PUT(sp.streams_forced); PUT(0); PUT(0); PUT(0);
     for (uint32_t i = 0; i < LNN_MAXCLS; i++) PUT(i < cc.nlen ? cc.lens[i] : 0);
     for (uint32_t i = 0; i < LNN_MAXCLS; i++) PUT(i < cc.nlen ? cc.slot_of[i] : 0);
+    }
     for (uint32_t f0 = 0; f0 < num_frames; f0 += (uint32_t)sp.chunk) {
         const uint32_t Fc = (num_frames - f0 < sp.chunk) ? (num_frames - f0) : (uint32_t)sp.chunk;
         for (int fin = 0; fin < (af_iters ? 2 : 1); fin++) {
-            const LnnChunkIn in = { &hs, C, S, Fc, tab->cls, meta + f0, &knob, sp.use_sub, has_side != 0, af_iters, learning, fin != 0 };
+            const LnnChunkIn in = { &hs, C, S, Fc, tab->cls, meta + f0, &knob, sp.use_sub, has_side != 0, af_iters, learning, fin != 0, lnn_lev_room(sp.part_bytes, per_frame, Fc) };
             LnnChunkForms cf;
             lnn_chunk_forms(&in, &cf);
+            if (mode == 2) {
+                PUT(f0); PUT(Fc); PUT(fin); PUT(in.lev_room);
+                for (uint32_t l = 0; l < hs.L; l++) {
+                    const LnnLayerForms &lf = cf.layer[l];
+                    PUT(lf.lev_scratch); PUT(lf.sub_small); PUT(lf.lev_beside); PUT(lf.nlev);
+                    for (uint32_t i = 0; i < LNN_MAXT; i++) { const bool on = i < lf.nlev; const LnnLevLaunch &v = lf.lev[on ? i : 0]; PUT(on ? v.t : 0); PUT(on ? v.u : 0); PUT(on ? v.threads : 0); PUT(on ? v.ride : 0); PUT(on ? v.lds : 0); PUT(on ? v.scratch : 0); }
+                }
+                continue;
+            }
             RowRuns rr; lnn_build_runs(&rr, meta + f0, Fc, C * hs.R);
             PUT(f0); PUT(Fc); PUT((uint64_t)Fc * C * (fin ? 1u : hs.R)); PUT(fin); PUT(cf.fwd_loss_on); PUT(cf.fuse_cfg); PUT(cf.fuse_all); PUT(cf.last_layer_all);
             PUT(cf.prep_defer); PUT(cf.hist); PUT(cf.chain_sum); PUT(cf.chain_sum_wave); PUT(cf.cascade_walk); PUT(rr.mixed); PUT(rr.n); PUT(cf.present);
diff --git a/linne_amd/csrc/lnn_forms.h b/linne_amd/csrc/lnn_forms.h
--- a/linne_amd/csrc/lnn_forms.h
+++ b/linne_amd/csrc/lnn_forms.h
@@ -31,6 +31,10 @@
 #define LNN_LEV_MAXRIDE 3u
 #define LEV_LDS(np_) (sizeof(double) * 64 * (size_t)(2 * (np_) + 3))
 #define LEV_LDS_BUDGET ((size_t)160 * 1024)
+#define LNN_LEVS_LOW 8u
+#define LEVS_LDS(np_) (sizeof(double) * 64 * (size_t)((np_) + 2 + LNN_LEVS_LOW))
+#define LNN_LEV_SCRATCH_BYTES(J_, np_) ((((uint64_t)(J_) + 63u) / 64u) * ((uint64_t)(np_) + 1u) * 64u * sizeof(double))
+#define LNN_SUB_LDS ((size_t)8 * (2 * 32 * 65 + 2 * LNN_MAXT * 32))
 #define LNN_SUB_TILE_SMALL 16u
 #define LNN_SUB_SMALL_LDS ((size_t)8 * (2 * LNN_SUB_TILE_SMALL * 65 + 2 * LNN_MAXT * 32))
 #define LNN_LEV_BESIDE_MIN 32768u
@@ -76,6 +80,8 @@
     int lev_ride;
     int lev_beside;
     int lev_wave;
+    int lev_scratch;
+    int sub_small;
     int search_two;
     int search_job;
     int fir_small;
@@ -102,6 +108,8 @@
     k->lev_ride = lnn_env_int("LINNE_AMD_LEV_RIDE", 1);
     k->lev_wave = lnn_env_int("LINNE_AMD_LEV_WAVE", 1);
     k->lev_beside = lnn_env_int("LINNE_AMD_LEV_BESIDE", -1);
+    k->lev_scratch = lnn_env_int("LINNE_AMD_LEV_SCRATCH", 1);
+    k->sub_small = lnn_env_int("LINNE_AMD_SUB_SMALL", -1);
     k->search_two = lnn_env_int("LINNE_AMD_SEARCH_TWO", 1);
     k->search_job = lnn_env_int("LINNE_AMD_SEARCH_JOB", -1);
     k->fwd_loss = lnn_env_int("LINNE_AMD_FWD_LOSS", -1);
@@ -304,7 +312,7 @@
     return rows_form && (S & 3u) == 0 && (P0 == 2u || P0 == 4u);
 }
 
-struct LnnLevLaunch { uint32_t t, u, threads, ride; size_t lds; };
+struct LnnLevLaunch { uint32_t t, u, threads, ride; size_t lds; bool scratch; };
 struct LnnLayerForms {
     bool fir_spec;
     bool hist_layer, hist_all;
@@ -312,6 +320,8 @@
     bool lev_wave;
     bool lev_inline;
     bool lev_beside;
+    bool lev_scratch;
+    bool sub_small;
     uint32_t lev_carrier;
     uint32_t nlev; LnnLevLaunch lev[LNN_MAXT];
     bool last_layer;
@@ -335,7 +345,9 @@
     const DevClass *cls; const uint32_t *idx;
     const LnnKnobs *k; bool use_sub, has_side; uint32_t af_iters, learning;
     bool final_pass;
-};
+    uint64_t lev_room;
+};
+static inline uint64_t lnn_lev_room(uint64_t part_bytes, uint64_t per_frame, uint32_t Fc) { const uint64_t used = per_frame * Fc; return part_bytes > used ? part_bytes - used : 0; }
 
 static inline void lnn_chunk_forms(const LnnChunkIn *in, LnnChunkForms *cf)
 {
@@ -382,17 +394,23 @@
             uint32_t ride = LNN_MAXT;
             for (uint32_t t = 1, u = 2; u <= maxu && k.lev_ride; u <<= 1, t++)
                 if (LEV_LDS(P) + LNN_LEV_MAXRIDE * LEV_LDS(P / u) <= LEV_LDS_BUDGET) { ride = t; break; }
+            lf.lev_scratch = k.lev_scratch != 0 && P >= 128u && in->lev_room >= LNN_LEV_SCRATCH_BYTES(CF * hs.R, P);
+            const size_t lds0 = lf.lev_scratch ? LEVS_LDS(P) : LEV_LDS(P);
             const bool beside_size = k.lev_beside >= 0 ? (k.lev_beside != 0) : (LNN_LEV_BESIDE_DEFAULT && J >= LNN_LEV_BESIDE_MIN);
             lf.lev_beside = beside_size && lf.hist_layer && P == 128u && in->has_side && ride >= 2u && ride < LNN_MAXT
-                    && LEV_LDS(P / 2u) + LNN_LEV_MAXRIDE * LEV_LDS(P >> ride) <= LEV_LDS_BUDGET && LEV_LDS(P) + LNN_SUB_SMALL_LDS <= LEV_LDS_BUDGET;
+                    && LEV_LDS(P / 2u) + LNN_LEV_MAXRIDE * LEV_LDS(P >> ride) <= LEV_LDS_BUDGET && lds0 + LNN_SUB_SMALL_LDS <= LEV_LDS_BUDGET;
+            lf.sub_small = lf.lev_beside && (k.sub_small >= 0 ? k.sub_small != 0 : lds0 + LNN_SUB_LDS > LEV_LDS_BUDGET);
             lf.lev_inline = lf.lev_beside && k.lev_beside == 2;
             if (ride < LNN_MAXT) lf.lev_carrier = lf.lev_beside ? 1u : 0u;
             for (uint32_t t = 0, u = 1; u <= maxu && t < (ride < LNN_MAXT ? ride : LNN_MAXT); u <<= 1, t++) {
                 const bool carry = (t == lf.lev_carrier);
                 LnnLevLaunch &v = lf.lev[lf.nlev++];
                 v.t = t; v.u = u;
-                v.lds = LEV_LDS(P / u) + (carry ? LNN_LEV_MAXRIDE * LEV_LDS(P >> ride) : 0);
-                v.threads = carry ? 64 * (1 + LNN_LEV_MAXRIDE) : 64;
+                v.scratch = lf.lev_scratch && t == 0;
+                uint32_t nr = LNN_LEV_MAXRIDE;
+                if (carry && v.scratch) { while (nr > 1u && 2 * (LEVS_LDS(P) + nr * LEV_LDS(P >> ride)) > LEV_LDS_BUDGET) nr--; if (2 * (LEVS_LDS(P) + nr * LEV_LDS(P >> ride)) > LEV_LDS_BUDGET) nr = LNN_LEV_MAXRIDE; }
+                v.lds = (v.scratch ? LEVS_LDS(P) : LEV_LDS(P / u)) + (carry ? nr * LEV_LDS(P >> ride) : 0);
+                v.threads = carry ? 64 * (1 + nr) : 64;
                 v.ride = carry ? ride : (uint32_t)LNN_MAXT;
             }
         }
diff --git a/linne_amd/csrc/lnn_k_levinson.h b/linne_amd/csrc/lnn_k_levinson.h
--- a/linne_amd/csrc/lnn_k_levinson.h
+++ b/linne_amd/csrc/lnn_k_levinson.h
@@ -1,7 +1,8 @@
 #ifndef LNN_K_LEVINSON_H_INCLUDED
 #define LNN_K_LEVINSON_H_INCLUDED
 
-__device__ __forceinline__ void levinson_problem(const Plan &p, uint32_t layer, uint32_t t, uint32_t unit, double *lev_lds, uint32_t lane, uint32_t job0)
+template <bool SCR>
+__device__ __forceinline__ void levinson_problem(const Plan &p, uint32_t layer, uint32_t t, uint32_t unit, double *lev_lds, uint32_t lane, uint32_t job0, double *gscr = nullptr)
 {
     uint32_t job = job0 + lane;
     const bool inrange = job < p.J;
@@ -16,7 +17,12 @@
     const double *r = p.acorr + ((size_t)ajob * LNN_MAXT + t) * LNN_ACW + (size_t)unit * (np + 1);
     double *h = p.tcoef + ((size_t)job * LNN_MAXT + t) * LNN_MAXP + (size_t)unit * np;
     const bool last = (layer + 1 == p.L);
-    for (uint32_t i = 0; i <= np; i++) sr[(size_t)i * 64] = have ? r[i] : 0.0;
+    double *gr = gscr + lane;
+    if (SCR) {
+        for (uint32_t i = 0; i <= np; i++) { const double v = have ? r[i] : 0.0; gr[(size_t)i * 64] = v; if (i < LNN_LEVS_LOW) sr[(size_t)i * 64] = v; }
+        __builtin_amdgcn_s_waitcnt(0);
+    } else
+        for (uint32_t i = 0; i <= np; i++) sr[(size_t)i * 64] = have ? r[i] : 0.0;
     for (uint32_t i = 0; i < np + 2; i++) sa[(size_t)i * 64] = 0.0;
     double tail = 0.0; int tail_set = 0;
     const double r0 = sr[0] * (1.0 + reg);
@@ -27,9 +33,46 @@
         const double a1 = -r1 / r0;
         ek += r1 * a1;
         sa[0] = 1.0; sa[64] = a1;
+        double qa0 = 0.0, qa1 = 0.0, qa2 = 0.0, qa3 = 0.0, qa4 = 0.0, qa5 = 0.0, qa6 = 0.0, qa7 = 0.0;
+        double qb0 = 0.0, qb1 = 0.0, qb2 = 0.0, qb3 = 0.0, qb4 = 0.0, qb5 = 0.0, qb6 = 0.0, qb7 = 0.0;
+        double qc0 = 0.0, qc1 = 0.0, qc2 = 0.0, qc3 = 0.0, qc4 = 0.0, qc5 = 0.0, qc6 = 0.0, qc7 = 0.0;
+#define LEVS_LOAD(B_, b_) do { int32_t bb_ = (b_); bb_ = bb_ < 8 ? 8 : (bb_ > (int32_t)np ? (int32_t)np : bb_); const double *g_ = gr + (size_t)bb_ * 64; \
+            B_##0 = g_[0]; B_##1 = *(g_ - 64); B_##2 = *(g_ - 128); B_##3 = *(g_ - 192); B_##4 = *(g_ - 256); B_##5 = *(g_ - 320); B_##6 = *(g_ - 384); B_##7 = *(g_ - 448); __builtin_amdgcn_sched_barrier(0); } while (0)
+#define LEVS_USE(B_) do { const double a0 = pa[0], a1_ = pa[64], a2 = pa[128], a3 = pa[192], a4 = pa[256], a5 = pa[320], a6 = pa[384], a7 = pa[448]; \
+            const double m0 = a0 * B_##0, m1 = a1_ * B_##1, m2 = a2 * B_##2, m3 = a3 * B_##3, m4 = a4 * B_##4, m5 = a5 * B_##5, m6 = a6 * B_##6, m7 = a7 * B_##7; \
+            gamma += m0; gamma += m1; gamma += m2; gamma += m3; gamma += m4; gamma += m5; gamma += m6; gamma += m7; pa += 512; __builtin_amdgcn_sched_barrier(0); } while (0)
+        if (SCR) { LEVS_LOAD(qa, 2); LEVS_LOAD(qb, 2 - 8); LEVS_LOAD(qc, 2 - 16); }
         for (uint32_t k = 1; k < np; k++) {
             double gamma = 0.0;
-            {
+            if (SCR) {
+                const double *pa = sa;
+                const uint32_t trips = (k + 1) >> 3;
+                uint32_t j = 0;
+                int32_t b = (int32_t)k + 1 - 24;
+                for (; j + 6 <= trips; j += 3, b -= 24) {
+                    LEVS_USE(qa); LEVS_LOAD(qa, b);
+                    LEVS_USE(qb); LEVS_LOAD(qb, b - 8);
+                    LEVS_USE(qc); LEVS_LOAD(qc, b - 16);
+                }
+                switch (trips - j) {
+                    case 5: LEVS_USE(qa); LEVS_LOAD(qa, b); LEVS_USE(qb); LEVS_LOAD(qb, b - 8); LEVS_USE(qc); LEVS_USE(qa); LEVS_USE(qb); break;
+                    case 4: LEVS_USE(qa); LEVS_LOAD(qa, b); LEVS_USE(qb); LEVS_USE(qc); LEVS_USE(qa); break;
+                    case 3: LEVS_USE(qa); LEVS_USE(qb); LEVS_USE(qc); break;
+                    case 2: LEVS_USE(qa); LEVS_USE(qb); break;
+                    case 1: LEVS_USE(qa); break;
+                    default: break;
+                }
+                uint32_t i = trips << 3;
+                const double *pr = sr + (size_t)(k + 1 - i) * 64;
+                for (; i + 4 <= k + 1; i += 4) {
+                    const double a0 = pa[0], a1_ = pa[64], a2 = pa[128], a3 = pa[192];
+                    const double q0 = pr[0], q1 = *(pr - 64), q2 = *(pr - 128), q3 = *(pr - 192);
+                    gamma += a0 * q0; gamma += a1_ * q1; gamma += a2 * q2; gamma += a3 * q3;
+                    pa += 256; pr -= 256;
+                }
+                for (; i <= k; i++) { gamma += pa[0] * pr[0]; pa += 64; pr -= 64; }
+                LEVS_LOAD(qa, (int32_t)k + 2); LEVS_LOAD(qb, (int32_t)k + 2 - 8); LEVS_LOAD(qc, (int32_t)k + 2 - 16);
+            } else {
                 const double *pa = sa, *pr = sr + (size_t)(k + 1) * 64;
                 uint32_t i = 0;
                 for (; i + 8 <= k + 1; i += 8) {
@@ -72,6 +115,8 @@
             sa[0] = a0n; sa[(size_t)(k + 1) * 64] = ak1;
             if (last && k == P0) { tail = -gamma; tail_set = 1; }
         }
+#undef LEVS_LOAD
+#undef LEVS_USE
     }
     if (!have) return;
     if (zero) {
@@ -88,18 +133,34 @@
 }
 
 #define LEV_MAXRIDE 3
-__global__ __launch_bounds__(64 * (1 + LEV_MAXRIDE)) void k_levinson_lds(Plan p, uint32_t layer, uint32_t t, uint32_t ride)
-{
-    extern __shared__ __attribute__((aligned(16))) double lev_lds[];
-    const uint32_t wave = threadIdx.x >> 6, lane = threadIdx.x & 63u, job0 = blockIdx.x * 64;
-    if (wave == 0) { levinson_problem(p, layer, t, blockIdx.y, lev_lds, lane, job0); return; }
+__device__ __forceinline__ void levinson_riders(const Plan &p, uint32_t layer, uint32_t ride, double *mine, uint32_t wave, uint32_t lane, uint32_t job0)
+{
     const uint32_t nride = (blockDim.x >> 6) - 1u, nseat = nride * gridDim.y, seat = blockIdx.y * nride + (wave - 1u);
-    double *mine = lev_lds + (size_t)(2 * (p.P[layer] >> t) + 3) * 64 + (size_t)(wave - 1u) * (2 * (p.P[layer] >> ride) + 3) * 64;
+    mine += (size_t)(wave - 1u) * (2 * (p.P[layer] >> ride) + 3) * 64;
     const uint32_t maxu = p.P[layer] < (uint32_t)LNN_MAXU ? p.P[layer] : (uint32_t)LNN_MAXU;
     uint32_t q = 0;
     for (uint32_t tt = ride, u = 1u << ride; u <= maxu; tt++, u <<= 1)
         for (uint32_t unit = 0; unit < u; unit++, q++)
-            if (q % nseat == seat) levinson_problem(p, layer, tt, unit, mine, lane, job0);
+            if (q % nseat == seat) levinson_problem<false>(p, layer, tt, unit, mine, lane, job0);
+}
+
+__global__ __launch_bounds__(64 * (1 + LEV_MAXRIDE)) void k_levinson_lds(Plan p, uint32_t layer, uint32_t t, uint32_t ride)
+{
+    extern __shared__ __attribute__((aligned(16))) double lev_lds[];
+    const uint32_t wave = threadIdx.x >> 6, lane = threadIdx.x & 63u, job0 = blockIdx.x * 64;
+    if (wave == 0) { levinson_problem<false>(p, layer, t, blockIdx.y, lev_lds, lane, job0); return; }
+    levinson_riders(p, layer, ride, lev_lds + (size_t)(2 * (p.P[layer] >> t) + 3) * 64, wave, lane, job0);
+}
+
+__global__ __launch_bounds__(64 * (1 + LEV_MAXRIDE)) void k_levinson_scr(Plan p, uint32_t layer, uint32_t t, uint32_t ride)
+{
+    extern __shared__ __attribute__((aligned(16))) double lev_lds[];
+    const uint32_t wave = threadIdx.x >> 6, lane = threadIdx.x & 63u, job0 = blockIdx.x * 64, np = p.P[layer] >> t;
+    if (wave == 0) {
+        levinson_problem<true>(p, layer, t, blockIdx.y, lev_lds, lane, job0, p.lev_scr + ((size_t)blockIdx.y * gridDim.x + blockIdx.x) * (size_t)(np + 1) * 64);
+        return;
+    }
+    levinson_riders(p, layer, ride, lev_lds + (size_t)(np + 2 + LNN_LEVS_LOW) * 64, wave, lane, job0);
 }
 
 __global__ __launch_bounds__(64) void k_levinson_wave(Plan p, uint32_t layer)
```
